# AbnerVictor/OOD-GAN-inversion

Hardware: AMD Instinct MI355X
Metric: 1024² face inversions/sec (100 W+ steps) (higher is better)
Workload: dtype f16-split (hi+lo f16 operands, f32 accumulate): 3 MFMA/product in every forward conv (fp32-equivalent), 2 in the input-gradient convs (back-propagated gradient rounded to f16 before each contraction, weights keep hi+lo); dL/dW+ vs the float64 reference 1.4e-5..3.6e-5 ('f16s': 1.3e-5..2.6e-5, the ref

## Files before the change

include/oodgan.h:

```cpp
#ifndef OODGAN_H
#define OODGAN_H

#ifdef __cplusplus
extern "C" {
#endif

#define OODGAN_OK 0
#define OODGAN_E_ARG (-1)
#define OODGAN_E_LAUNCH (-2)
#define OODGAN_E_STATE (-3)
#define OODGAN_E_NODEV (-4)

int oodgan_version(void);
const char* oodgan_last_error(void);
int oodgan_device_count(void);
int oodgan_set_tunable(const char* name, long value);
long oodgan_get_tunable(const char* name);
long oodgan_dispatch_count(const char* name);
int oodgan_dispatch_reset(void);
int oodgan_zero(void* p, long bytes, void* stream);

void* oodgan_plan_create(void);
int oodgan_plan_destroy(void* plan);
int oodgan_plan_record_begin(void* plan);
// ... 100 lines not shown
    const float* noise_w;
    const float* bias;
    const float* dscale;
    const float* mul2;
    void* ys;
    float* part_r;
    float* part_t;
    float* part_max;
    int s_rgb_stride, noise_batch, dscale_stride;
    float rgb_scale;
    long nmax;
    int ys_hi_only;
} oodgan_actbwd_fuse;

int oodgan_conv3x3(const oodgan_conv_args* args, void* stream);

long oodgan_pack_conv3x3_f16s_bytes(int Co, int Ci, int transpose);
int oodgan_pack_conv3x3_f16s(const float* w, void* wpk16, float* unscale2, int Co, int Ci, float scale, int transpose,
                             int flip, void* stream);
int oodgan_conv3x3_f16s(const oodgan_conv_args* args, const float* unscale2, void* stream);
int oodgan_conv3x3_f16s_nparts(int mode, int Hin, int Win);
int oodgan_conv3x3_f16s_nparts2(int mode, int Hin, int Win, int x_sform);
int oodgan_conv3x3_s2_fuse_supported(int B, int K, int M, int Hin, int Win);
int oodgan_conv3x3_s2_grouped_supported(int B, int K, int M, int groups, int Hin, int Win);
int oodgan_conv3x3_s1_actgrad_supported(int B, int K, int M, int H, int W);
int oodgan_conv3x3_s1_ys_supported(int B, int K, int M, int H, int W);
int oodgan_conv3x3_xf_supported(int B, int K, int M, int H, int W);
int oodgan_conv3x3_xf_nparts(int B, int H, int W);
long oodgan_conv3x3_tiny_workspace(int mode, int B, int K, int M, int Hin, int Win);

#define OODGAN_VMAX_SLOTS 64
long oodgan_sform_bytes(int B, int C, int H, int W);
int oodgan_to_sform(const float* x, const float* scale, int scale_stride, const float* shift, int shift_stride,
                    const float* mul2, void* out, int B, int C, int H, int W, int in_pitch, unsigned* vmax, void* stream);
long oodgan_sform_phases_bytes(int B, int C, int H, int W);
int oodgan_from_sform(const void* xs, const float* scale, int scale_stride, float* y, int B, int C, int H, int W, void* stream);
int oodgan_blurT_to_sform_phases(const float* g, const float* kernel, const float* scale, int scale_stride,
                                 const float* mul2, void* out, int B, int C, int H, int W, void* stream);
int oodgan_to_sform_phases(const float* x, const float* scale, int scale_stride, const float* mul2, void* out, int B,
                           int C, int H, int W, int in_pitch, void* stream);
int oodgan_to_sform_phases_padtl(const float* x, const float* scale, int scale_stride, const float* mul2, void* out, int B,
                                 int C, int H, int W, int in_pitch, void* stream);
int oodgan_conv3x3_nparts(int mode, int Hin, int Win);
int oodgan_absmax_scaled(const float* x, const float* s, int s_stride, unsigned* vmax, int B, int C, long HW, void* stream);
int oodgan_fwd_range_update(unsigned* vmax, float* q, int* flag, int n, void* stream);
int oodgan_fwd_range_plan(const float* s_all, const float* d_all, const int* row_layer, const int* drow_layer, const float* q,
                          float* s_sc, float* d_sc, int B, int R, int DR, int row0, int nrows, int drow0, int ndrows,
                          void* stream);

int oodgan_blur_act_sform(const float* z, const float* kernel, float* y, void* ys, const float* ys_scale, int ys_scale_stride,
                          const float* bias, const float* noise, int noise_batch, const float* noise_w, int act, int B, int C,
                          int H, int W, int in_pitch, unsigned* vmax, void* stream);
int oodgan_blur_act_fform(const float* z, const float* kernel, float* y, const float* ys_scale, int ys_scale_stride,
                          const float* bias, const float* noise, int noise_batch, const float* noise_w, int act,
                          int B, int C, int H, int W, int in_pitch, unsigned* vmax, int kernel_rank_one, void* stream);
int oodgan_upconv_vblur_supported(int B, int K, int M, int H, int W);
int oodgan_upconv_vblur_fform(const void* xs, const void* wpk2, long wset_bytes, const float* unscale4, const float* kh4,
                              const float* out_scale, int out_scale_stride, const float* bias, const float* noise, int noise_batch,
                              const float* noise_w, int act, const float* ys_scale, int ys_scale_stride, unsigned* vmax, float* y,
                              int B, int K, int M, int H, int W, void* stream);
int oodgan_blur_act_sform_sep(const float* z, const float* kernel, float* y, void* ys, const float* ys_scale, int ys_scale_stride,
                              const float* bias, const float* noise, int noise_batch, const float* noise_w, int act, int B, int C,
                              int H, int W, int in_pitch, unsigned* vmax, int kernel_rank_one, void* stream);

int oodgan_act_bwd_sform_nparts(int H, int W);
int oodgan_act_bwd_sform(const float* g_feat, const float* out, const float* noise, int noise_batch, const float* noise_w,
                         const float* bias, const float* g_rgb, const float* w_rgb, const float* s_rgb, int s_rgb_stride,
                         float rgb_scale, const float* dscale, int dscale_stride, const float* mul2, void* ys, float* part_r,
                         float* part_t, float* part_max, int B, int C, int H, int W, void* stream);
int oodgan_act_bwd_sform_f(const float* out_f, const float* noise, int noise_batch, const float* noise_w, const float* bias,
                           const float* g_rgb, const float* w_rgb, const float* s_rgb, int s_rgb_stride, float rgb_scale,
                           const float* dscale, int dscale_stride, const float* mul2, void* ys, float* part_r, float* part_t,
                           float* part_max, int B, int C, int H, int W, void* stream);
int oodgan_from_fform(const float* f, float* y, int B, int C, int H, int W, void* stream);
int oodgan_act_bwd_blurT_nparts(int H, int W);
int oodgan_act_bwd_blurT_pre_supported(int H, int W);
int oodgan_act_bwd_blurT_sform_phases(const float* g_feat, const float* out, const float* noise, int noise_batch,
                                      const float* noise_w, const float* bias, const float* g_rgb, const float* w_rgb,
                                      const float* s_rgb, int s_rgb_stride, float rgb_scale, const float* dscale,
                                      int dscale_stride, const float* mul2, const float* kernel, void* out_phases,
                                      float* part_r, float* part_t, float* part_max, int B, int C, int H, int W, void* stream);
int oodgan_act_bwd_blurT_hi_supported(int H, int W);
int oodgan_conv3x3_s1_xh_supported(int B, int K, int M, int H, int W);
int oodgan_act_bwd_blurT_sform_phases_hi(const float* g_feat, const float* out, const float* noise, int noise_batch, const float* noise_w,
                                         const float* bias, const float* dscale, int dscale_stride, const float* mul2, const float* kernel,
                                         void* out_phases, float* part_r, float* part_max, int B, int C, int H, int W, void* stream);
int oodgan_absmax_scale_check(const float* part, long n, float* state, int* flag, void* stream);

typedef struct oodgan_reduce_job {
    const float* part;
    float* out;
    int B, C, nparts, out_stride, accumulate;
    const float* part2;
    const float* scale2;
    int nparts2, scale2_stride;
} oodgan_reduce_job;
typedef struct oodgan_demod_bwd_job {
    const float* s; const float* wsq; const float* d; const float* r; float* gs;
    int s_stride, d_stride, gs_stride, B, Ci, Co;
    float scale;
} oodgan_demod_bwd_job;
typedef struct oodgan_demod_fwd_job {
    const float* s; const float* wsq; float* d;
    int s_stride, d_stride, B, Ci, Co;
    float scale;
} oodgan_demod_fwd_job;
typedef struct oodgan_scale_check_job {
    const float* part; long n; float* state;
} oodgan_scale_check_job;
int oodgan_reduce_batch(const oodgan_reduce_job* jobs, int njobs, void* stream);
int oodgan_demod_bwd_batch(const oodgan_demod_bwd_job* jobs, int njobs, void* stream);
int oodgan_demod_fwd_batch(const oodgan_demod_fwd_job* jobs, int njobs, void* stream);
int oodgan_absmax_scale_check_batch(const oodgan_scale_check_job* jobs, int njobs, int* flag, void* stream);

long oodgan_hform_bytes(int B, int C, int H, int W);
int oodgan_to_hform(const float* x, void* out, int B, int C, int H, int W, void* stream);
int oodgan_from_hform(const void* in, float* y, int B, int C, int H, int W, void* stream);
long oodgan_modconv_f16_wbytes(int B, int M, int K);
int oodgan_modconv_f16_pack(const float* weight, const float* style, int style_stride, float scale, int demodulate,
                            int act, void* wpk, int B, int M, int K, void* stream);
int oodgan_modconv_f16_pack_affine(const float* weight, const float* latent, int latent_stride, const float* mod_weight,
                                   const float* mod_bias, int S, float scale, int demodulate, int act, void* wpk, int B, int M,
                                   int K, void* stream);
int oodgan_modconv_f16(const void* x, const void* wpk, const float* noise, int noise_batch, const float* noise_w,
                       const float* bias, int act, void* y, int B, int K, int M, int H, int W, void* stream);
int oodgan_reduce_parts(const float* part, float* out, long rows, int nparts, int accumulate, void* stream);
int oodgan_reduce_parts_cols(const float* part, float* out, int B, int C, int nparts, int out_stride, int accumulate,
                             void* stream);


int oodgan_torgb_fwd(const float* x, const float* w, const float* s, int s_stride, const float* bias,
                     const float* skip, const float* kernel, float* y, int B, int Ci, int H, int W,
                     float scale, void* stream);
int oodgan_torgb_fwd_sform(const float* x, const float* w, const float* s, int s_stride, const float* bias,
                           const float* skip, const float* kernel, float* y, void* ys, const float* ys_scale,
                           int ys_scale_stride, int B, int Ci, int H, int W, float scale, unsigned* vmax, void* stream);
int oodgan_rgb_finish(const float* partial, const float* bias, const float* skip, const float* kernel, float* y, int B, int H,
                      int W, void* stream);
int oodgan_rgb_finish_parts(const float* partial, int nparts, const float* bias, const float* skip, const float* kernel, float* y, int B,
                            int H, int W, void* stream);

int oodgan_feature_modulation(const float* x, const float* c0, const float* c1, float* y, long n, int mode, void* stream);

int oodgan_act_bwd_fused(const float* g_feat, const float* out, const float* noise, int noise_batch,
                         const float* noise_w, const float* bias, const float* g_rgb, const float* w_rgb,
                         const float* s_rgb, int s_rgb_stride, float rgb_scale, float* g_pre,
                         float* part_r, float* part_rgb, int B, int C, long HW, void* stream);
int oodgan_act_bwd_nparts(long HW);
int oodgan_act_bwd_fused_max(const float* g_feat, const float* out, const float* noise, int noise_batch,
                             const float* noise_w, const float* bias, const float* g_rgb, const float* w_rgb,
                             const float* s_rgb, int s_rgb_stride, float rgb_scale, float* g_pre,
                             float* part_r, float* part_rgb, float* part_max, const float* dscale, int dscale_stride, int B,
                             int C, long HW, void* stream);
int oodgan_absmax_scale(const float* part, long n, float* out2, void* stream);
int oodgan_absmax_scale_clear(float* part, long n, float* out2, void* stream);


int oodgan_mse_fwd_bwd(const float* img, const float* target, float* gimg, float* part, float* loss,
                       int B, long CHW, float grad_mul, void* stream);
int oodgan_mse_nparts(long CHW);
int oodgan_mse_fwd_bwd_row(const float* img, const float* target, float* gimg, float* part, float* loss_table,
                           const int* row_dev, int nrows, int B, long CHW, float grad_mul, void* stream);
int oodgan_composite_mse_fwd_bwd(const float* img, const float* target, const float* beta, float* gimg, float* comp, float* part,
                                 float* loss, int B, int C, long HW, int wrt_gen, float grad_mul, void* stream);
int oodgan_composite_mse_fwd_bwd_row(const float* img, const float* target, const float* beta, float* gimg, float* comp, float* part,
                                     float* loss_table, const int* row_dev, int nrows, int B, int C, long HW, int wrt_gen,
// ... 83 lines not shown
```

ood-gan-inversion_amd/csrc/common.hpp:

```cpp
#pragma once
#include <hip/hip_runtime.h>
#include <cstdio>
#include <cstdarg>
#include <functional>
#include <utility>
#include "../../include/oodgan.h"

namespace oodgan {
struct PlanRec;
extern thread_local PlanRec* tl_plan_rec;
extern int g_null_launch;
void plan_append(std::function<void()>&& f);
template <class F>
inline void launch_rec(F&& f) {
    f();
    if (__builtin_expect(tl_plan_rec != nullptr, 0)) plan_append(std::function<void()>(std::forward<F>(f)));
}
}
#undef hipLaunchKernelGGL
#define hipLaunchKernelGGL(kernelName, numBlocks, numThreads, memPerBlock, streamId, ...)                                        \
    ::oodgan::launch_rec([=]() {                                                                                                 \
        if (!::oodgan::g_null_launch) (kernelName)<<<(numBlocks), (numThreads), (memPerBlock), (streamId)>>>(__VA_ARGS__);      \
    })

namespace oodgan {

void set_error(const char* fmt, ...);

enum { OODGAN_TUN_S1_BIG_MIN_ITEMS = 0, OODGAN_TUN_S2_BIG_MIN_ITEMS, OODGAN_TUN_T2_BIG_MIN_ITEMS, OODGAN_TUN_BLURT_STRIP, OODGAN_TUN_BLUR_STRIP, OODGAN_TUN_UPVB_WAVES, OODGAN_TUN_FEWOUT_QUAD, OODGAN_TUN_TINY_MID_MAX, OODGAN_TUN_STRIPX_WAVES, OODGAN_TUN_COUNT };
long tunable(int id);

enum { OODGAN_DC_STRIPX = 0, OODGAN_DC_STRIP, OODGAN_DC_S1BIG, OODGAN_DC_S1V2, OODGAN_DC_S1PP, OODGAN_DC_TINY, OODGAN_DC_T2BIG,
       OODGAN_DC_T2V2, OODGAN_DC_T2GEN, OODGAN_DC_S2BIG, OODGAN_DC_S2V2, OODGAN_DC_S2GEN, OODGAN_DC_UPVB,
       OODGAN_DC_S1BIG_YS, OODGAN_DC_S2BIG_FUSE, OODGAN_DC_S2BIG_DOTXS,
       OODGAN_DC_S1BIG_G2, OODGAN_DC_S2BIG_G2, OODGAN_DC_STRIPX_G2, OODGAN_DC_S2BIG_XH, OODGAN_DC_S1BIG_XH,
       OODGAN_DC_COMPOSITE_MSE,
       OODGAN_DC_SSIM,
       OODGAN_DC_ROBUST,
       OODGAN_DC_AREA_POOL, OODGAN_DC_COUNT };
void count_dispatch(int id);

bool bound_device_ok(const char* what);

inline int check_launch(const char* what) {
    hipError_t e = hipGetLastError();
    if (e != hipSuccess) {
        set_error("%s: %s", what, hipGetErrorString(e));
        return OODGAN_E_LAUNCH;
    }
    return OODGAN_OK;
}

#define OODGAN_REQUIRE(cond, ...)          \
    do {                                    \
        if (!(cond)) {                      \
            oodgan::set_error(__VA_ARGS__); \
            return OODGAN_E_ARG;            \
        }                                   \
    } while (0)

constexpr float kSqrt2 = 1.4142135623730951f;
constexpr float kInvPos = 1.f / kSqrt2, kInvNeg = 1.f / (0.2f * kSqrt2);
constexpr int kWave = 64;

inline hipStream_t as_stream(void* s) { return reinterpret_cast<hipStream_t>(s); }

inline int stream_grid(long work_items, int block) {
    long g = (work_items + block - 1) / block;
    if (g > 2048) g = 2048;
    if (g < 1) g = 1;
    return static_cast<int>(g);
}

__device__ __forceinline__ float wave_sum(float v) {
#pragma unroll
    for (int o = 32; o > 0; o >>= 1) v += __shfl_xor(v, o, 64);
    return v;
}

__device__ __forceinline__ float row_sum16(const float* __restrict__ p, int n, int l) {
    float v[4];
#pragma unroll
    for (int u = 0; u < 4; ++u) v[u] = p[min(l + 16 * u, n - 1)];
#pragma unroll
    for (int u = 0; u < 4; ++u) v[u] = l + 16 * u < n ? v[u] : 0.f;
    float r = (v[0] + v[1]) + (v[2] + v[3]);
    r += __shfl_xor(r, 8, 64);
    r += __shfl_xor(r, 4, 64);
    r += __shfl_xor(r, 2, 64);
    r += __shfl_xor(r, 1, 64);
    return r;
}

__device__ __forceinline__ float row_sum_wave(const float* __restrict__ p, int n, int lane) {
    float a0 = 0.f, a1 = 0.f, a2 = 0.f, a3 = 0.f;
    for (int i0 = lane; i0 < n; i0 += 512) {
        float v[8];
#pragma unroll
        for (int u = 0; u < 8; ++u) v[u] = p[min(i0 + 64 * u, n - 1)];
#pragma unroll
        for (int u = 0; u < 8; ++u) v[u] = i0 + 64 * u < n ? v[u] : 0.f;
        a0 += v[0] + v[4]; a1 += v[1] + v[5]; a2 += v[2] + v[6]; a3 += v[3] + v[7];
    }
    return wave_sum((a0 + a1) + (a2 + a3));
}

__device__ __forceinline__ float row_sum(const float* __restrict__ p, int n, int lane) {
    return n <= 64 ? row_sum16(p, n, lane & 15) : row_sum_wave(p, n, lane);
}

__device__ __forceinline__ float demod_dot(const float* __restrict__ sp, const float* __restrict__ wp, int Ci, int lane) {
    float a0 = 0.f, a1 = 0.f, a2 = 0.f, a3 = 0.f;
    for (int c0 = lane; c0 < Ci; c0 += 512) {
        float sv[8], wv[8];
#pragma unroll
        for (int u = 0; u < 8; ++u) {
            const int ci = min(c0 + 64 * u, Ci - 1);
            sv[u] = sp[ci];
            wv[u] = wp[ci];
        }
#pragma unroll
        for (int u = 0; u < 8; ++u) {
// ... 78 lines not shown
```

ood-gan-inversion_amd/csrc/conv_f16s.hip:

```cpp
#include "conv_common.hpp"
#include <cstdlib>
#include <cstdint>

extern "C" int oodgan_conv3x3_f16s_nparts(int mode, int Hin, int Win);

using namespace oodgan;

namespace oodgan {
int launch_s1pp(const oodgan_conv_args& a, const void* wpk16, const float* unscale, hipStream_t st);
int launch_s1v2(const oodgan_conv_args& a, const void* wpk16, const float* unscale, hipStream_t st);
bool s1_strip_eligible(const oodgan_conv_args& a);
bool s1_big_eligible(const oodgan_conv_args& a);
int launch_s1_big(const oodgan_conv_args& a, const void* wpk16, const float* unscale, hipStream_t st);
int launch_s1_strip(const oodgan_conv_args& a, const void* wpk16, const float* unscale, hipStream_t st);
int launch_s1_stripx(const oodgan_conv_args& a, const void* wpk16, const float* unscale, hipStream_t st);
bool tiny_eligible(const oodgan_conv_args& a);
int launch_tiny(const oodgan_conv_args& a, const void* wpk16, const float* unscale, hipStream_t st);
int launch_t2v2(const oodgan_conv_args& a, const void* wpk16, const float* unscale, hipStream_t st);
int launch_s2v2(const oodgan_conv_args& a, const void* wpk16, const float* unscale, hipStream_t st);
bool s2_big_eligible(const oodgan_conv_args& a);
bool t2_big_eligible(const oodgan_conv_args& a);
int launch_t2_big(const oodgan_conv_args& a, const void* wpk16, const float* unscale, hipStream_t st);
int launch_s2_big(const oodgan_conv_args& a, const void* wpk16, const float* unscale, hipStream_t st);
}
// ... 311 lines not shown
}

__global__ __launch_bounds__(256) void pack_f16s_kernel(const float* __restrict__ w, _Float16* __restrict__ out, int Co, int Ci,
                                                        int Mp, float scale, int transpose, int flip,
                                                        const float* __restrict__ sc2) {
    const int K = transpose ? Co : Ci, M = transpose ? Ci : Co;
    const int nchunk = (K + CK - 1) / CK;
    const long total = (long)nchunk * 9 * 2 * Mp * 8;
    const float s2 = sc2[1] * scale;
    for (long e = blockIdx.x * 256L + threadIdx.x; e < total; e += (long)gridDim.x * 256) {
        const int j = (int)(e & 7);
        long r = e >> 3;
        const int m = (int)(r % Mp); r /= Mp;
        const int h = (int)(r & 1); r >>= 1;
        const int tap = (int)(r % 9);
        const int t = (int)(r / 9);
        const int k = t * CK + 8 * h + j;
        float v = 0.f;
        if (m < M && k < K) {
            const int co = transpose ? k : m, ci = transpose ? m : k;
            v = w[((long)co * Ci + ci) * 9 + (flip ? 8 - tap : tap)] * s2;
        }
        const _Float16 hi = (_Float16)v;
        const _Float16 lo = (_Float16)(v - (float)hi);
        const long base = (((long)t * 9 + tap) * 2) * 2;
        out[((base + 0 * 2 + h) * Mp + m) * 8 + j] = hi;
        out[((base + 1 * 2 + h) * Mp + m) * 8 + j] = lo;
    }
}

}

extern "C" int oodgan_conv3x3_f16s_nparts2(int mode, int Hin, int Win, int x_sform) {
    if (mode == OODGAN_CONV_S2 && x_sform) return (((Hin - 1) / 2 + 7) / 8) * (((Win - 1) / 2 + 31) / 32);
    return oodgan_conv3x3_f16s_nparts(mode, Hin, Win);
}

extern "C" int oodgan_conv3x3_f16s_nparts(int mode, int Hin, int Win) {
    if (mode == OODGAN_CONV_S1) return ((Hin + 7) / 8) * ((Win + 31) / 32) ;
    if (mode == OODGAN_CONV_S2) return (((Hin - 1) / 2 + 7) / 8) * (((Win - 1) / 2 + 31) / 32) * 4;
    return 0;
}

extern "C" long oodgan_pack_conv3x3_f16s_bytes(int Co, int Ci, int transpose) {
    const int M = transpose ? Ci : Co, K = transpose ? Co : Ci;
    const long Mp = (M + 63) / 64 * 64;
    return (long)((K + CK - 1) / CK) * 9 * 2 * 2 * Mp * 16;
}

extern "C" int oodgan_pack_conv3x3_f16s(const float* w, void* wpk16, float* unscale2, int Co, int Ci, float scale, int transpose,
                                        int flip, void* stream) {
    OODGAN_REQUIRE(w && wpk16 && unscale2 && Co > 0 && Ci > 0, "pack_conv3x3_f16s: bad args");
    const int M = transpose ? Ci : Co, K = transpose ? Co : Ci;
    const int Mp = (M + 63) / 64 * 64;
    hipStream_t st = as_stream(stream);
    if (hipMemsetAsync(unscale2, 0, 2 * sizeof(float), st) != hipSuccess) {
        set_error("pack_conv3x3_f16s: memset failed");
        return OODGAN_E_LAUNCH;
    }
    hipLaunchKernelGGL(absmax_kernel, dim3(stream_grid((long)Co * Ci * 9, 256 * 16)), dim3(256), 0, st, w, (long)Co * Ci * 9, scale, unscale2);
    hipLaunchKernelGGL(absmax_finish_kernel, dim3(1), dim3(1), 0, st, unscale2);
    const long total = (long)((K + CK - 1) / CK) * 9 * 2 * Mp * 8;
    hipLaunchKernelGGL(pack_f16s_kernel, dim3(stream_grid(total, 256)), dim3(256), 0, st, w, reinterpret_cast<_Float16*>(wpk16),
                       Co, Ci, Mp, scale, transpose, flip, unscale2);
    return check_launch("pack_conv3x3_f16s");
}

extern "C" int oodgan_conv3x3_s1_actgrad_supported(int B, int K, int M, int H, int W) {
    oodgan_conv_args a = {};
    a.mode = OODGAN_CONV_S1; a.x_sform = 1; a.B = B; a.K = K; a.M = M; a.Hin = H; a.Win = W;
    a.y = reinterpret_cast<float*>(1);
    a.dotx = reinterpret_cast<const float*>(1);
    return (s1_strip_eligible(a) || s1_big_eligible(a)) && oodgan_act_bwd_blurT_pre_supported(H / 2, W / 2) && !(H & 1) && !(W & 1) ? 1 : 0;
}

extern "C" int oodgan_conv3x3_s1_xh_supported(int B, int K, int M, int H, int W) {
    oodgan_conv_args a = {};
    a.mode = OODGAN_CONV_S1; a.x_sform = 1; a.B = B; a.K = K; a.M = M; a.Hin = H; a.Win = W;
    a.y = reinterpret_cast<float*>(1);
    a.dotx = reinterpret_cast<const float*>(1);
    return (H > 8 && W > 8 && !s1_strip_eligible(a) && s1_big_eligible(a)) ? 1 : 0;
}

extern "C" int oodgan_conv3x3_s1_ys_supported(int B, int K, int M, int H, int W) {
    oodgan_conv_args a = {};
    a.mode = OODGAN_CONV_S1; a.x_sform = 1; a.B = B; a.K = K; a.M = M; a.Hin = H; a.Win = W;
    a.ys = reinterpret_cast<void*>(1);
    return s1_big_eligible(a) ? 1 : 0;
}

extern "C" int oodgan_conv3x3_f16s(const oodgan_conv_args* args, const float* unscale2, void* stream) {
    OODGAN_REQUIRE(args != nullptr, "conv3x3_f16s: null args");
    const oodgan_conv_args& a = *args;
    OODGAN_REQUIRE(a.x && a.wpk && unscale2 && (a.y || a.x_sform), "conv3x3_f16s: null tensor");
    OODGAN_REQUIRE(a.B > 0 && a.K > 0 && a.M > 0 && a.Hin > 0 && a.Win > 0, "conv3x3_f16s: bad shape");
    OODGAN_REQUIRE(a.act != OODGAN_ACT_PRELU || a.slope, "conv3x3_f16s: PReLU without slopes");
    OODGAN_REQUIRE(a.noise == nullptr || a.noise_batch == 1 || a.noise_batch == a.B, "conv3x3_f16s: noise_batch");
    if (!bound_device_ok("conv3x3_f16s")) return OODGAN_E_ARG;
    if (a.x_fform) {
        OODGAN_REQUIRE(a.x_fform == 1 || a.x_fform == 2, "conv3x3_f16s: x_fform must be 0, 1 or 2");
        count_dispatch(OODGAN_DC_STRIPX);
        return launch_s1_stripx(a, a.wpk, unscale2, as_stream(stream));
    }
    OODGAN_REQUIRE(!a.dotx_fform, "conv3x3_f16s: an F-form dotx exists only with x_fform == 2");
    OODGAN_REQUIRE(a.rgb_y == nullptr || (a.mode == OODGAN_CONV_S1 && a.x_sform), "conv3x3_f16s: fused ToRGB output only for mode S1 with S-form input");
    OODGAN_REQUIRE(a.fuse == nullptr || (a.mode == OODGAN_CONV_S2 && a.x_sform && a.M >= 64),
                   "conv3x3_f16s: the fused activation backward exists only for mode S2 with S-form input and M >= 64");
    OODGAN_REQUIRE(a.groups <= 1 || (a.mode == OODGAN_CONV_S2 && (!a.x_sform || tiny_eligible(a) || s2_big_eligible(a))),
                   "conv3x3_f16s: groups > 1 only for mode S2 with fp32 NCHW input, or a phase-split S-form input of a shape the 8-wave or the skinny-GEMM kernel "
                   "takes (oodgan_conv3x3_s2_grouped_supported; oodgan_conv3x3_tiny_workspace > 0 with a workspace)");
    OODGAN_REQUIRE(!a.y_fform || (a.mode == OODGAN_CONV_S1 && a.x_sform && s1_strip_eligible(a)),
                   "conv3x3_f16s: the F-form output exists only in the strip kernel (mode S1, S-form input, 16 < K,M <= 32)");
    OODGAN_REQUIRE(!a.dot_actgrad || (a.mode == OODGAN_CONV_S1 && a.x_sform && a.dotx && (s1_strip_eligible(a) || s1_big_eligible(a))),
                   "conv3x3_f16s: dot_actgrad exists only in the strip / 8-wave kernels of mode S1 (oodgan_conv3x3_s1_actgrad_supported)");
    OODGAN_REQUIRE(!a.dotx_sform || (a.mode == OODGAN_CONV_S2 && a.x_sform && a.fuse && a.dotx && a.dotx_scale && a.dotx_scale_stride >= a.M &&
                                     !tiny_eligible(a) && s2_big_eligible(a)),
                   "conv3x3_f16s: dotx_sform needs mode S2, a phase-split S-form input, `fuse`, dotx, dotx_scale and a shape of the 8-wave kernel "
                   "(oodgan_conv3x3_s2_fuse_supported)");
    OODGAN_REQUIRE(a.ys_vmax == nullptr || (a.ys != nullptr && a.mode == OODGAN_CONV_S1 && a.x_sform && !tiny_eligible(a) && !s1_strip_eligible(a) && s1_big_eligible(a)),
                   "conv3x3_f16s: ys_vmax only with ys from the 8-wave stride-1 kernel (oodgan_conv3x3_s1_ys_supported)");
    OODGAN_REQUIRE(a.x_hi_only != 2 || (a.x_sform && a.dotx && !tiny_eligible(a) &&
                                        ((a.mode == OODGAN_CONV_S2 && s2_big_eligible(a)) || (a.mode == OODGAN_CONV_S1 && !s1_strip_eligible(a) && s1_big_eligible(a)))),
                   "conv3x3_f16s: x_hi_only = 2 (32-byte hi-only input records) exists only in the two-instruction 8-wave kernels (S-form input, dotx; mode S2 on a "
                   "shape oodgan_conv3x3_s2_fuse_supported accepts, mode S1 on a shape of the 8-wave stride-1 kernel)");
    hipStream_t st = as_stream(stream);
    switch (a.mode) {
        case OODGAN_CONV_S1:
            if (tiny_eligible(a)) { count_dispatch(OODGAN_DC_TINY); return launch_tiny(a, a.wpk, unscale2, st); }
            if (a.x_sform && s1_strip_eligible(a)) { count_dispatch(OODGAN_DC_STRIP); return launch_s1_strip(a, a.wpk, unscale2, st); }
            if (a.x_sform && s1_big_eligible(a)) { count_dispatch(OODGAN_DC_S1BIG); if (a.ys) count_dispatch(OODGAN_DC_S1BIG_YS); return launch_s1_big(a, a.wpk, unscale2, st); }
            OODGAN_REQUIRE(a.rgb_y == nullptr, "conv3x3_f16s: the fused ToRGB output exists only in the strip kernel (16 < K,M <= 32) and, as partial "
                                               "sums together with ys, in the 8-wave kernel (oodgan_conv3x3_s1_ys_supported)");
            if (a.x_sform) { count_dispatch(OODGAN_DC_S1V2); return launch_s1v2(a, a.wpk, unscale2, st); }
            OODGAN_REQUIRE(a.ys == nullptr, "conv3x3_f16s: S-form output needs the S-form input kernel");
            count_dispatch(OODGAN_DC_S1PP);
            return launch_s1pp(a, a.wpk, unscale2, st);
        case OODGAN_CONV_T2:
            if (a.x_sform && t2_big_eligible(a)) { count_dispatch(OODGAN_DC_T2BIG); return launch_t2_big(a, a.wpk, unscale2, st); }
            if (a.x_sform) { count_dispatch(OODGAN_DC_T2V2); return launch_t2v2(a, a.wpk, unscale2, st); }
            count_dispatch(OODGAN_DC_T2GEN);
            return launch_mode<OODGAN_CONV_T2>(a, a.wpk, unscale2, st);
        case OODGAN_CONV_S2:
            OODGAN_REQUIRE((a.Hin & 1) && (a.Win & 1) && a.Hin >= 3 && a.Win >= 3, "conv3x3_f16s S2: input must be odd-sized");
            if (tiny_eligible(a)) { count_dispatch(OODGAN_DC_TINY); return launch_tiny(a, a.wpk, unscale2, st); }
            if (a.x_sform && s2_big_eligible(a)) { count_dispatch(OODGAN_DC_S2BIG); if (a.fuse) count_dispatch(OODGAN_DC_S2BIG_FUSE); if (a.dotx_sform) count_dispatch(OODGAN_DC_S2BIG_DOTXS); return launch_s2_big(a, a.wpk, unscale2, st); }
            if (a.x_sform) { count_dispatch(OODGAN_DC_S2V2); return launch_s2v2(a, a.wpk, unscale2, st); }
            count_dispatch(OODGAN_DC_S2GEN);
            return launch_mode<OODGAN_CONV_S2>(a, a.wpk, unscale2, st);
        default: break;
    }
    set_error("conv3x3_f16s: unknown mode %d", a.mode);
    return OODGAN_E_ARG;
}
```

ood-gan-inversion_amd/csrc/conv_f16s_big.hip:

```cpp
#include "conv_common.hpp"
#include "sform.hpp"
#include <cstdint>
#include <cstdlib>
#include <type_traits>

using namespace oodgan;

typedef _Float16 half8 __attribute__((ext_vector_type(8)));
typedef __attribute__((address_space(3))) void lds_void;

namespace {

constexpr int BG_R = 18, BG_C = 34;
constexpr int BG_XSLOTS = BG_R * BG_C * 4;
constexpr int BG_XPIECES = (BG_XSLOTS + 63) / 64;
constexpr int BG_XBYTES = BG_XPIECES * 1024;
constexpr int BG_WPIECES = 36;
constexpr int BG_STAGE = BG_XBYTES + BG_WPIECES * 1024;
constexpr int BG_PIECES = BG_XPIECES + BG_WPIECES;
constexpr int BG_RED = 2 * BG_STAGE;
constexpr int BG_SMEM = BG_RED + 8 * 64 * 4;

struct BigConv {
    oodgan_conv_args a;
    const uint4* xs;
    SDims xd;
    const float* w_unscale;
    int tiles_x, tiles_y, mblocks, Mp;
    long out_plane;
    SDims yd;
};

constexpr int BG_ZERO = BG_SMEM;
constexpr int BG_ZBYTES = 3584;
constexpr int BG_CST = BG_SMEM + BG_ZBYTES;
constexpr int BG_NZ = BG_CST + 3 * 64 * 4;
constexpr int BG_RGBW = BG_NZ + 2048;
constexpr int BG_SMEM16 = BG_RGBW + 3 * 64 * 4;
typedef float f32x4v __attribute__((ext_vector_type(4)));

#ifdef OODGAN_CLOCK_STAMP
__device__ unsigned long long* g_s1big_stamp = nullptr;
__device__ long g_s1big_stamp_n = 0;
#endif

template <bool DOT, bool PRE, bool YS = false, bool G2 = false>
__global__ __launch_bounds__(512) void conv_f16s_s1big_kernel(const BigConv p, const uint4* __restrict__ wpk16) {
    constexpr int NW = 8, NT = 2;
    extern __shared__ __attribute__((aligned(16))) unsigned char smem[];
    const oodgan_conv_args& a = p.a;
    const int tid = threadIdx.x, lane = tid & 63;
    const int wave = __builtin_amdgcn_readfirstlane(tid >> 6);
    const int n16 = lane & 15, g = lane >> 4;

    int w = xcd_remap(blockIdx.x, gridDim.x);
    const int mblk = w % p.mblocks;
    w /= p.mblocks;
    const int ntile = p.tiles_x * p.tiles_y;
    const int tile = w % ntile, b = w / ntile;
    const int ty = tile / p.tiles_x, tx = tile % p.tiles_x;
    const int r0 = ty * 16, c0 = tx * 32, m0 = mblk * 64;
    const int H = a.Hin, W = a.Win, M = a.M;

    constexpr int NPW = (BG_PIECES + NW - 1) / NW;
    unsigned off[NPW];
    const bool xh = G2 && a.x_hi_only == 2;
    unsigned xmask = 0;
    const int KC = p.xd.KC;
#pragma unroll
    for (int i = 0; i < NPW; ++i) {
        const int pc = wave + NW * i;
        if (pc < BG_XPIECES) {
            int P = pc * 64 + lane;
            if (P >= BG_XSLOTS) P = BG_XSLOTS - 1;
            const int row = P / (BG_C * 4), q = P % (BG_C * 4);
            const int c = q >> 2, sl = ((q & 3) - 2 * ((c >> 2) & 1)) & 3;
            const int rr = min(r0 + row, p.xd.Hp - 1);
            if (xh) {
                off[i] = (unsigned)((((long)rr * p.xd.Wp + (c0 + c)) * 2 + (sl & 1)) * 16);
                if (sl < 2) xmask |= 1u << i;
            } else {
                off[i] = (unsigned)((((long)rr * p.xd.Wp + (c0 + c)) * 4 + sl) * 16);
                xmask |= 1u << i;
            }
        } else {
            xmask |= 1u << i;
            const int u = (pc - BG_XPIECES) * 64 + lane;
            const int row = u >> 6, j = u & 63;
            off[i] = (unsigned)((((long)row * p.Mp) + m0 + j) * 16);
        }
    }
    const unsigned char* xb = reinterpret_cast<const unsigned char*>(p.xs) + (long)b * KC * p.xd.plane * 16;
    const long xplane_bytes = p.xd.plane * 16;
    const unsigned char* wb = reinterpret_cast<const unsigned char*>(wpk16);
    const long wchunk_bytes = (long)36 * p.Mp * 16;
    const int nchunk = (a.K + 15) / 16;
    auto dma_piece = [&](int t, int buf, int i) {
        const int pc = wave + NW * i;
        if (pc >= BG_PIECES) return;
        unsigned char* dst = smem + buf * BG_STAGE;
        const unsigned char* src = (pc < BG_XPIECES ? xb + (long)t * xplane_bytes : wb + (long)t * wchunk_bytes) + off[i];
        if (!G2 || ((xmask >> i) & 1u))
            __builtin_amdgcn_global_load_lds((const __attribute__((address_space(1))) void*)src, (lds_void*)(dst + pc * 1024), 16, 0, 0);
    };
    for (int i = tid; i < BG_ZBYTES / 16; i += 512) reinterpret_cast<uint4*>(smem + BG_ZERO)[i] = make_uint4(0, 0, 0, 0);
    __syncthreads();

    f32x4v acc[4][4];
#pragma unroll
    for (int mt = 0; mt < 4; ++mt)
#pragma unroll
        for (int n = 0; n < 4; ++n) acc[mt][n] = f32x4v{0.f, 0.f, 0.f, 0.f};

    const unsigned laneA = (unsigned)((((g & 1) * 64 + n16) * 16) + (g >> 1) * 4096);
    const unsigned laneA1 = (unsigned)(((g & 1) * 64 + n16) * 16);
    unsigned offBh[4], offBl[4];
#pragma unroll
    for (int pp = 0; pp < 4; ++pp) {
        const int tp = 2 * pp + (g >> 1), ky = tp / 3, kx = tp % 3, col = n16 + kx;
        offBh[pp] = (unsigned)(ky * (BG_C * 64) + col * 64 + ((((g & 1) + 2 * ((col >> 2) & 1)) & 3) << 4));
        offBl[pp] = (unsigned)(ky * (BG_C * 64) + col * 64 + ((((g & 1) + 2 + 2 * ((col >> 2) & 1)) & 3) << 4));
    }
    const int col8 = n16 + 2;
    const unsigned offB1 = (unsigned)(2 * (BG_C * 64) + col8 * 64 + ((((G2 ? (g & 1) : g) + 2 * ((col8 >> 2) & 1)) & 3) << 4));

    struct AF { half8 x[2], y[2]; };
    struct BF { half8 u[4], v[4]; };
    auto load_a = [&](AF& f, const unsigned char* lw, auto pp_c, auto mh_c) {
        constexpr int pp = decltype(pp_c)::value, mh = decltype(mh_c)::value;
        const unsigned char* q = lw + (pp < 4 ? laneA + 2 * pp * 4096 : laneA1 + 8 * 4096 + (G2 ? (g >> 1) * 2048 : 0));
#pragma unroll
        for (int i = 0; i < 2; ++i) {
            f.x[i] = *reinterpret_cast<const half8*>(q + (2 * mh + i) * 256);
            if (!(G2 && pp == 4)) f.y[i] = *reinterpret_cast<const half8*>(q + 2048 + (2 * mh + i) * 256);
        }
    };
    auto load_b = [&](BF& f, const unsigned char* lx, const unsigned char* lz, auto pp_c, auto part_c) {
        constexpr int pp = decltype(pp_c)::value, part = decltype(part_c)::value;
#pragma unroll
        for (int n = 0; n < 4; ++n) {
            const int o = (n >> 1) * (BG_C * 64) + (n & 1) * 1024;
            if (G2) {
                if (part == 0) f.u[n] = *reinterpret_cast<const half8*>(lx + (pp < 4 ? offBh[pp < 4 ? pp : 0] : offB1) + o);
            } else if (pp < 4) {
                if (part == 0) f.u[n] = *reinterpret_cast<const half8*>(lx + offBh[pp < 4 ? pp : 0] + o);
                else f.v[n] = *reinterpret_cast<const half8*>(lx + offBl[pp < 4 ? pp : 0] + o);
            } else {
                if (part == 0) f.u[n] = *reinterpret_cast<const half8*>(lx + offB1 + o);
                else f.v[n] = *reinterpret_cast<const half8*>(lz + o);
            }
        }
    };
    auto mfma_half = [&](const AF& fa, const BF& fb, auto pp_c, auto mh_c) {
        constexpr int pp = decltype(pp_c)::value, mh = decltype(mh_c)::value;
        if (G2) {
#pragma unroll
            for (int i = 0; i < 2; ++i)
#pragma unroll
                for (int n = 0; n < 4; ++n) acc[2 * mh + i][n] = __builtin_amdgcn_mfma_f32_16x16x32_f16(fa.x[i], fb.u[n], acc[2 * mh + i][n], 0, 0, 0);
            if (pp < 4) {
#pragma unroll
                for (int i = 0; i < 2; ++i)
#pragma unroll
                    for (int n = 0; n < 4; ++n) acc[2 * mh + i][n] = __builtin_amdgcn_mfma_f32_16x16x32_f16(fa.y[i], fb.u[n], acc[2 * mh + i][n], 0, 0, 0);
            }
        } else if (pp < 4) {
#pragma unroll
            for (int i = 0; i < 2; ++i)
#pragma unroll
                for (int n = 0; n < 4; ++n) acc[2 * mh + i][n] = __builtin_amdgcn_mfma_f32_16x16x32_f16(fa.x[i], fb.u[n], acc[2 * mh + i][n], 0, 0, 0);
#pragma unroll
            for (int i = 0; i < 2; ++i)
#pragma unroll
                for (int n = 0; n < 4; ++n) acc[2 * mh + i][n] = __builtin_amdgcn_mfma_f32_16x16x32_f16(fa.x[i], fb.v[n], acc[2 * mh + i][n], 0, 0, 0);
#pragma unroll
            for (int i = 0; i < 2; ++i)
#pragma unroll
                for (int n = 0; n < 4; ++n) acc[2 * mh + i][n] = __builtin_amdgcn_mfma_f32_16x16x32_f16(fa.y[i], fb.u[n], acc[2 * mh + i][n], 0, 0, 0);
        } else {
#pragma unroll
            for (int i = 0; i < 2; ++i)
#pragma unroll
                for (int n = 0; n < 4; ++n) acc[2 * mh + i][n] = __builtin_amdgcn_mfma_f32_16x16x32_f16(fa.x[i], fb.u[n], acc[2 * mh + i][n], 0, 0, 0);
#pragma unroll
            for (int i = 0; i < 2; ++i)
#pragma unroll
                for (int n = 0; n < 4; ++n) acc[2 * mh + i][n] = __builtin_amdgcn_mfma_f32_16x16x32_f16(fa.y[i], fb.v[n], acc[2 * mh + i][n], 0, 0, 0);
        }
    };
#define BH_IC(n) std::integral_constant<int, n>{}
#define BH_SB() __builtin_amdgcn_sched_barrier(0)
#ifdef OODGAN_CLOCK_STAMP
    const unsigned long long st_t0 = __builtin_amdgcn_s_memtime(), st_r0 = __builtin_amdgcn_s_memrealtime();
#endif
    float cst_o = 0.f, cst_b = 0.f, cst_s = 1.f, rgb_c0 = 0.f, rgb_c1 = 0.f, rgb_c2 = 0.f;
    if (tid < 64 && m0 + tid < M) {
        const int m = m0 + tid;
        cst_o = a.out_scale ? a.out_scale[(long)b * a.out_scale_stride + m] : 1.f;
        if (!DOT && a.bias) cst_b = a.bias[m];
        if (!DOT && a.act == OODGAN_ACT_PRELU) cst_s = a.slope[m];
        if (YS && a.rgb_y) {
            const float sv = a.rgb_scale * a.rgb_s[(long)b * a.rgb_s_stride + m];
            rgb_c0 = sv * a.rgb_w[m]; rgb_c1 = sv * a.rgb_w[M + m]; rgb_c2 = sv * a.rgb_w[2 * M + m];
        }
    }
    const bool has_nz = !DOT && a.noise != nullptr;
    if (has_nz) {
        const int ry = min(r0 + wave * NT + (lane >> 5), H - 1), rx = min(c0 + (lane & 31), W - 1);
        const float* src = a.noise + (long)(a.noise_batch > 1 ? b : 0) * H * W + (long)ry * W + rx;
        __builtin_amdgcn_global_load_lds((const __attribute__((address_space(1))) void*)src, (lds_void*)(smem + BG_NZ + wave * 256), 4, 0, 0);
    }
#pragma unroll
    for (int i = 0; i < NPW; ++i) dma_piece(0, 0, i);
    if (tid < 64) {
        float* cst = reinterpret_cast<float*>(smem + BG_CST);
        cst[tid] = cst_o;
        if (!DOT) { cst[64 + tid] = cst_b; cst[128 + tid] = cst_s; }
        if (YS) {
            float* rw = reinterpret_cast<float*>(smem + BG_RGBW);
            rw[tid] = rgb_c0; rw[64 + tid] = rgb_c1; rw[128 + tid] = rgb_c2;
        }
        __builtin_amdgcn_s_waitcnt(0xC07F);
    }
    for (int t = 0; t < nchunk; ++t) {
        __builtin_amdgcn_s_waitcnt(0x0F70);
        __builtin_amdgcn_s_barrier();
        const bool pf = t + 1 < nchunk;
        const int nb = (t + 1) & 1;
        const unsigned char* lx = smem + (t & 1) * BG_STAGE + (wave * NT) * (BG_C * 64);
        const unsigned char* lw = smem + (t & 1) * BG_STAGE + BG_XBYTES;
        const unsigned col8r = (unsigned)(2 * (BG_C * 64) + col8 * 64 + ((((g & 1) + 2 * ((col8 >> 2) & 1)) & 3) << 4));
        const unsigned char* lz = g < 2 ? lx + col8r : smem + BG_ZERO;
        AF a0, a1;
        BF b0, b1;
#define BH_DMA(i) if (pf && (i) < NPW) dma_piece(t + 1, nb, (i));
        load_b(b0, lx, lz, BH_IC(0), BH_IC(0)); load_b(b0, lx, lz, BH_IC(0), BH_IC(1));
        load_a(a0, lw, BH_IC(0), BH_IC(0));
        BH_SB();
        load_a(a1, lw, BH_IC(0), BH_IC(1)); load_b(b1, lx, lz, BH_IC(1), BH_IC(0)); BH_DMA(0) BH_SB(); mfma_half(a0, b0, BH_IC(0), BH_IC(0)); BH_SB();
        load_a(a0, lw, BH_IC(1), BH_IC(0)); load_b(b1, lx, lz, BH_IC(1), BH_IC(1)); BH_DMA(1) BH_SB(); mfma_half(a1, b0, BH_IC(0), BH_IC(1)); BH_SB();
        load_a(a1, lw, BH_IC(1), BH_IC(1)); load_b(b0, lx, lz, BH_IC(2), BH_IC(0)); BH_DMA(2) BH_SB(); mfma_half(a0, b1, BH_IC(1), BH_IC(0)); BH_SB();
        load_a(a0, lw, BH_IC(2), BH_IC(0)); load_b(b0, lx, lz, BH_IC(2), BH_IC(1)); BH_DMA(3) BH_SB(); mfma_half(a1, b1, BH_IC(1), BH_IC(1)); BH_SB();
        load_a(a1, lw, BH_IC(2), BH_IC(1)); load_b(b1, lx, lz, BH_IC(3), BH_IC(0)); BH_DMA(4) BH_SB(); mfma_half(a0, b0, BH_IC(2), BH_IC(0)); BH_SB();
        load_a(a0, lw, BH_IC(3), BH_IC(0)); load_b(b1, lx, lz, BH_IC(3), BH_IC(1)); BH_DMA(5) BH_SB(); mfma_half(a1, b0, BH_IC(2), BH_IC(1)); BH_SB();
        load_a(a1, lw, BH_IC(3), BH_IC(1)); load_b(b0, lx, lz, BH_IC(4), BH_IC(0)); BH_DMA(6) BH_SB(); mfma_half(a0, b1, BH_IC(3), BH_IC(0)); BH_SB();
        load_a(a0, lw, BH_IC(4), BH_IC(0)); load_b(b0, lx, lz, BH_IC(4), BH_IC(1)); BH_DMA(7) BH_SB(); mfma_half(a1, b1, BH_IC(3), BH_IC(1)); BH_SB();
        load_a(a1, lw, BH_IC(4), BH_IC(1)); BH_DMA(8) BH_SB(); mfma_half(a0, b0, BH_IC(4), BH_IC(0)); BH_SB();
        BH_DMA(9) BH_SB();
        mfma_half(a1, b0, BH_IC(4), BH_IC(1));
#undef BH_DMA
    }
#undef BH_IC
#undef BH_SB
#ifdef OODGAN_CLOCK_STAMP
    if (tid == 0 && g_s1big_stamp && (long)blockIdx.x < g_s1big_stamp_n) {
        g_s1big_stamp[2 * blockIdx.x] = __builtin_amdgcn_s_memtime() - st_t0;
        g_s1big_stamp[2 * blockIdx.x + 1] = __builtin_amdgcn_s_memrealtime() - st_r0;
    }
#endif

    const float us = (p.w_unscale ? p.w_unscale[0] : 1.f) * (a.in_mul2 ? a.in_mul2[0] : 1.f);
    const float nw = (!DOT && a.noise) ? (a.noise_w ? a.noise_w[0] : 1.f) : 0.f;
    float* red = reinterpret_cast<float*>(smem + BG_RED);
    float osc[16], bia[16], slp[16];
    unsigned moff[16], doff[16];
    float dsum[16];
    const bool prelu = !DOT && a.act == OODGAN_ACT_PRELU;
    const float* cst = reinterpret_cast<const float*>(smem + BG_CST);
#pragma unroll
    for (int q = 0; q < 16; ++q) {
        const int j = 16 * (q >> 2) + 4 * g + (q & 3), m = m0 + j;
        const bool mok = m < M;
        osc[q] = cst[j] * us;
        bia[q] = DOT ? 0.f : cst[64 + j];
        slp[q] = DOT ? 1.f : cst[128 + j];
        moff[q] = mok ? (unsigned)((long)m * p.out_plane * 4) : 0xFFFFFFFFu;
        doff[q] = mok ? (unsigned)((long)m * H * W * 4) : 0u;
        dsum[q] = 0.f;
    }
    const bool mfull = m0 + 64 <= M;
    float ysc[16], ysmax = 0.f;
    if (YS) {
#pragma unroll
        for (int q = 0; q < 16; ++q) {
            const int m = m0 + 16 * (q >> 2) + 4 * g + (q & 3);
            ysc[q] = a.ys_scale ? a.ys_scale[(long)b * a.ys_scale_stride + min(m, M - 1)] : 1.f;
        }
    }
#pragma unroll
    for (int n = 0; n < 4; ++n) {
        const int py = r0 + wave * NT + (n >> 1), px = c0 + 16 * (n & 1) + n16;
        const bool ok = py < H && px < W;
        float nz = 0.f;
        if (has_nz) nz = nw * reinterpret_cast<const float*>(smem + BG_NZ)[wave * 64 + (n >> 1) * 32 + 16 * (n & 1) + n16];
        unsigned char* yr = reinterpret_cast<unsigned char*>(a.y) + ((long)b * M * p.out_plane + (long)py * a.out_pitch + px) * 4;
        const unsigned char* dr = DOT ? reinterpret_cast<const unsigned char*>(a.dotx) + ((long)b * M * H * W + (long)py * W + px) * 4 : nullptr;
        float o[16], dv[16];
        if (DOT) {
#pragma unroll
            for (int q = 0; q < 16; ++q) dv[q] = 0.f;
            if (ok) {
                if (mfull) {
#pragma unroll
                    for (int q = 0; q < 16; ++q) dv[q] = *reinterpret_cast<const float*>(dr + doff[q]);
                } else {
#pragma unroll
                    for (int q = 0; q < 16; ++q)
                        if (moff[q] != 0xFFFFFFFFu) dv[q] = *reinterpret_cast<const float*>(dr + doff[q]);
                }
            }
        }
#pragma unroll
        for (int q = 0; q < 16; ++q) {
            const float v = acc[q >> 2][n][q & 3];
            o[q] = v * osc[q];
            if (DOT) {
                dsum[q] += (v * us) * dv[q];
                if (PRE) o[q] *= dv[q] > 0.f ? kSqrt2 : 0.2f * kSqrt2;
            } else {
                o[q] += nz + bia[q];
                if (a.act == OODGAN_ACT_LRELU) o[q] = (o[q] > 0.f ? o[q] : 0.2f * o[q]) * kSqrt2;
                else if (prelu) o[q] = o[q] > 0.f ? o[q] : slp[q] * o[q];
            }
        }
        if (ok && (!YS || a.y != nullptr)) {
            if (mfull) {
#pragma unroll
                for (int q = 0; q < 16; ++q) *reinterpret_cast<float*>(yr + moff[q]) = o[q];
            } else {
#pragma unroll
                for (int q = 0; q < 16; ++q)
                    if (moff[q] != 0xFFFFFFFFu) *reinterpret_cast<float*>(yr + moff[q]) = o[q];
            }
        }
        if (YS && !DOT && ok) {
#pragma unroll
            for (int mt = 0; mt < 4; ++mt) {
                if (m0 + 16 * mt < M) {
                    const float v0 = o[4 * mt] * ysc[4 * mt], v1 = o[4 * mt + 1] * ysc[4 * mt + 1], v2 = o[4 * mt + 2] * ysc[4 * mt + 2],
                                v3 = o[4 * mt + 3] * ysc[4 * mt + 3];
                    ysmax = fmaxf(fmaxf(ysmax, fmaxf(fabsf(v0), fabsf(v1))), fmaxf(fabsf(v2), fabsf(v3)));
                    uint2 hi, lo;
                    split_pair(v0, v1, hi.x, lo.x);
                    split_pair(v2, v3, hi.y, lo.y);
                    unsigned char* rec = reinterpret_cast<unsigned char*>(a.ys) + sform_unit(p.yd, b, (m0 >> 4) + mt, py, px, g >> 1) * 16 + (g & 1) * 8;
                    *reinterpret_cast<uint2*>(rec) = hi;
                    *reinterpret_cast<uint2*>(rec + 32) = lo;
                }
            }
        }
        if (YS && !DOT && a.rgb_y) {
            const float* rw = reinterpret_cast<const float*>(smem + BG_RGBW);
            float c0 = 0.f, c1 = 0.f, c2 = 0.f;
#pragma unroll
            for (int q = 0; q < 16; ++q) {
                const int j = 16 * (q >> 2) + 4 * g + (q & 3);
                c0 += rw[j] * o[q]; c1 += rw[64 + j] * o[q]; c2 += rw[128 + j] * o[q];
            }
            c0 += __shfl_xor(c0, 16, 64); c1 += __shfl_xor(c1, 16, 64); c2 += __shfl_xor(c2, 16, 64);
            c0 += __shfl_xor(c0, 32, 64); c1 += __shfl_xor(c1, 32, 64); c2 += __shfl_xor(c2, 32, 64);
            if (ok && g == 0) {
                float* rp = a.rgb_y + (((long)mblk * a.B + b) * 3) * ((long)H * W) + (long)py * W + px;
                rp[0] = c0; rp[(long)H * W] = c1; rp[2 * (long)H * W] = c2;
            }
        }
    }
    if (YS && a.ys_vmax) record_vmax(a.ys_vmax, b, ysmax);
    if (DOT) {
#pragma unroll
        for (int q = 0; q < 16; ++q) {
            float v = dsum[q];
            v += dpp_take<0xB1, 0xF>(v);
            v += dpp_take<0x4E, 0xF>(v);
            v += dpp_take<0x141, 0xF>(v);
            v += dpp_take<0x140, 0xF>(v);
            if (n16 == 0) red[wave * 64 + 16 * (q >> 2) + 4 * g + (q & 3)] = v;
        }
        __syncthreads();
        if (tid < 64 && m0 + tid < M) {
            float v = 0.f;
#pragma unroll
            for (int wv = 0; wv < NW; ++wv) v += red[wv * 64 + tid];
            float* dp = a.dot_part + ((long)b * M + m0 + tid) * a.dot_nparts;
            const int tx8 = (W + 31) / 32;
            dp[(long)(2 * ty) * tx8 + tx] = v;
            if (2 * ty + 1 < (H + 7) / 8) dp[(long)(2 * ty + 1) * tx8 + tx] = 0.f;
        }
    }
}

}

namespace oodgan {

bool s1_big_eligible(const oodgan_conv_args& a) {
    const int min_k = 64;
    if (!(a.mode == OODGAN_CONV_S1 && a.x_sform && a.K >= min_k && a.M >= 64 && (a.ys == nullptr ? (a.y != nullptr && a.rgb_y == nullptr) : (a.dotx == nullptr && a.M % 16 == 0)) &&
          (a.act == OODGAN_ACT_NONE || a.act == OODGAN_ACT_LRELU || (a.act == OODGAN_ACT_PRELU && a.slope)) && a.in_scale == nullptr &&
          a.in_shift == nullptr &&
          !(a.dotx && (a.noise || a.bias || a.act != OODGAN_ACT_NONE))))
        return false;
    const long items = (long)((a.Hin + 15) / 16) * ((a.Win + 31) / 32) * a.B * ((a.M + 63) / 64);
    return items >= tunable(OODGAN_TUN_S1_BIG_MIN_ITEMS);
}

int launch_s1_big(const oodgan_conv_args& a_in, const void* wpk16, const float* unscale, hipStream_t st) {
    BigConv p;
    p.a = a_in;
    oodgan_conv_args& a = p.a;
    if (a.out_pitch == 0) a.out_pitch = a.Win;
    p.out_plane = (long)a.Hin * a.out_pitch;
    p.xs = reinterpret_cast<const uint4*>(a.x);
    p.xd = sform_dims(a.K, a.Hin, a.Win);
    p.w_unscale = unscale;
    p.tiles_y = (a.Hin + 15) / 16;
    p.tiles_x = (a.Win + 31) / 32;
    p.Mp = (a.M + 63) / 64 * 64;
    p.mblocks = (a.M + 63) / 64;
    p.yd = sform_dims(a.M, a.Hin, a.Win);
    if (a.dotx) {
        OODGAN_REQUIRE(a.dot_part != nullptr, "conv3x3: dotx without dot_part");
        OODGAN_REQUIRE(a.dot_nparts == ((a.Hin + 7) / 8) * p.tiles_x, "conv3x3 f16s S1: dot_nparts %d != %d", a.dot_nparts,
                       ((a.Hin + 7) / 8) * p.tiles_x);
    }
    OODGAN_REQUIRE((long)a.M * p.out_plane * 4 < (1L << 32) && (long)a.M * a.Hin * a.Win * 4 < (1L << 32), "conv3x3 big: plane too large");
    const long total = (long)p.tiles_x * p.tiles_y * a.B * p.mblocks;
    OODGAN_REQUIRE(total > 0 && total < (1L << 31), "conv3x3: grid too large");
    static bool once = ((void)hipFuncSetAttribute(reinterpret_cast<const void*>(&conv_f16s_s1big_kernel<true, false>), hipFuncAttributeMaxDynamicSharedMemorySize, BG_SMEM16),
                        (void)hipFuncSetAttribute(reinterpret_cast<const void*>(&conv_f16s_s1big_kernel<true, true>), hipFuncAttributeMaxDynamicSharedMemorySize, BG_SMEM16),
                        (void)hipFuncSetAttribute(reinterpret_cast<const void*>(&conv_f16s_s1big_kernel<false, false>), hipFuncAttributeMaxDynamicSharedMemorySize, BG_SMEM16),
                        (void)hipFuncSetAttribute(reinterpret_cast<const void*>(&conv_f16s_s1big_kernel<false, false, true>), hipFuncAttributeMaxDynamicSharedMemorySize, BG_SMEM16),
                        (void)hipFuncSetAttribute(reinterpret_cast<const void*>(&conv_f16s_s1big_kernel<true, false, false, true>), hipFuncAttributeMaxDynamicSharedMemorySize, BG_SMEM16),
                        (void)hipFuncSetAttribute(reinterpret_cast<const void*>(&conv_f16s_s1big_kernel<true, true, false, true>), hipFuncAttributeMaxDynamicSharedMemorySize, BG_SMEM16), true);
    (void)once;
    const uint4* w16 = reinterpret_cast<const uint4*>(wpk16);
    OODGAN_REQUIRE(!a.dot_actgrad || a.dotx, "conv3x3 big: dot_actgrad without dotx");
    const bool g2 = a.x_hi_only != 0 && a.dotx != nullptr;
    OODGAN_REQUIRE(a.x_hi_only != 2 || g2, "conv3x3 big: hi-only input records (x_hi_only = 2) need dotx (the two-instruction instances)");
    if (g2) count_dispatch(OODGAN_DC_S1BIG_G2);
    if (g2 && a.x_hi_only == 2) count_dispatch(OODGAN_DC_S1BIG_XH);
    if (a.dot_actgrad && g2) hipLaunchKernelGGL((conv_f16s_s1big_kernel<true, true, false, true>), dim3((unsigned)total), dim3(512), BG_SMEM16, st, p, w16);
    else if (g2) hipLaunchKernelGGL((conv_f16s_s1big_kernel<true, false, false, true>), dim3((unsigned)total), dim3(512), BG_SMEM16, st, p, w16);
    else if (a.dot_actgrad) hipLaunchKernelGGL((conv_f16s_s1big_kernel<true, true>), dim3((unsigned)total), dim3(512), BG_SMEM16, st, p, w16);
    else if (a.dotx) hipLaunchKernelGGL((conv_f16s_s1big_kernel<true, false>), dim3((unsigned)total), dim3(512), BG_SMEM16, st, p, w16);
    else if (a.ys) hipLaunchKernelGGL((conv_f16s_s1big_kernel<false, false, true>), dim3((unsigned)total), dim3(512), BG_SMEM16, st, p, w16);
    else hipLaunchKernelGGL((conv_f16s_s1big_kernel<false, false>), dim3((unsigned)total), dim3(512), BG_SMEM16, st, p, w16);
    return check_launch("conv3x3_f16s_s1big");
}

}

#ifdef OODGAN_CLOCK_STAMP
extern "C" int oodgan_debug_set_stamp_buffer(void* buf, long n) {
    unsigned long long* p = reinterpret_cast<unsigned long long*>(buf);
    if (hipMemcpyToSymbol(HIP_SYMBOL(g_s1big_stamp), &p, sizeof(p)) != hipSuccess ||
        hipMemcpyToSymbol(HIP_SYMBOL(g_s1big_stamp_n), &n, sizeof(n)) != hipSuccess) {
        oodgan::set_error("debug_set_stamp_buffer: hipMemcpyToSymbol failed");
        return OODGAN_E_LAUNCH;
    }
    return 0;
}
#endif
```

ood-gan-inversion_amd/csrc/fwd_producers.hip:

```cpp
#include "common.hpp"
#include "sform.hpp"
#include <cstdint>

using namespace oodgan;

typedef _Float16 half2v __attribute__((ext_vector_type(2)));
typedef _Float16 half8 __attribute__((ext_vector_type(8)));

namespace {

constexpr int FT_R = 11, FT_C = 72;
constexpr int FT_P = 74, FT_Q = 816;
constexpr int LS_ROW = 65, LS_CH = 520;

__device__ __forceinline__ bool tile_elem(int k, int i, int& r, int& c4) {
    if (k < FT_R) { r = k; c4 = i; return true; }
    r = i; c4 = 16 + (k - FT_R);
    return i < FT_R;
}

struct BlurArgs {
    const float* z;
    const float* kern;
    float* y;
// ... 52 lines not shown
            const int gy = Y0 - 1 + r, gx = X0 - 4 + 4 * c4;
            v[k] = make_float4(0.f, 0.f, 0.f, 0.f);
            if (act && c < a.C && gy >= 0 && gy < Hz && gx >= 0 && gx + 3 < a.pitch)
                v[k] = *reinterpret_cast<const float4*>(zp + (long)gy * a.pitch + gx);
        }
#pragma unroll
        for (int k = 0; k < NE; ++k) {
            int r, c4;
            if (!tile_elem(k, tid & 15, r, c4)) continue;
            const int gx = X0 - 4 + 4 * c4;
            if (gx + 3 >= Wz) {
                if (gx + 0 >= Wz) v[k].x = 0.f;
                if (gx + 1 >= Wz) v[k].y = 0.f;
                if (gx + 2 >= Wz) v[k].z = 0.f;
                v[k].w = 0.f;
            }
            float2* dst = reinterpret_cast<float2*>(lin + ch * FT_Q + r * FT_P + 4 * c4);
            dst[0] = make_float2(v[k].x, v[k].y);
            dst[1] = make_float2(v[k].z, v[k].w);
        }
    }
    __syncthreads();
    const int ch = tid >> 4, tq = tid & 15;
    const int yrow = tq >> 1, xh = tq & 1;
    float o[32];
    if (ksep[8] != 0.f) {
#pragma unroll
        for (int hf = 0; hf < 2; ++hf) {
            float tmp[20];
#pragma unroll
            for (int j = 0; j < 20; ++j) tmp[j] = 0.f;
#pragma unroll
            for (int aa = 0; aa < 4; ++aa) {
                const float2* row = reinterpret_cast<const float2*>(lin + ch * FT_Q + (yrow + aa) * FT_P + 32 * xh + 16 * hf + 2);
                const float kv = ksep[aa];
#pragma unroll
                for (int j = 0; j < 10; ++j) {
                    const float2 v = row[j];
                    tmp[2 * j] += kv * v.x;
                    tmp[2 * j + 1] += kv * v.y;
                }
            }
#pragma unroll
            for (int j = 0; j < 16; ++j)
                o[16 * hf + j] = ksep[4] * tmp[j + 1] + ksep[5] * tmp[j + 2] + ksep[6] * tmp[j + 3] + ksep[7] * tmp[j + 4];
        }
    } else {
#pragma unroll
        for (int j = 0; j < 32; ++j) o[j] = 0.f;
#pragma unroll
        for (int aa = 0; aa < 4; ++aa) {
            const float* row = lin + ch * FT_Q + (yrow + aa) * FT_P + 32 * xh + 3;
            float win[35];
#pragma unroll
            for (int j = 0; j < 35; ++j) win[j] = row[j];
#pragma unroll
            for (int bb = 0; bb < 4; ++bb) {
                const float kv = kf[aa * 4 + bb];
#pragma unroll
                for (int j = 0; j < 32; ++j) o[j] += kv * win[j + bb];
            }
        }
    }
    __syncthreads();
    float* lst = lin;
#pragma unroll
    for (int j = 0; j < 32; ++j) lst[ch * LS_CH + yrow * LS_ROW + 32 * xh + j] = o[j];
    __syncthreads();
    const float nw = a.noise ? (a.noise_w ? a.noise_w[0] : 1.f) : 0.f;
    const long HWo = (long)Ho * Wo;
    float vm = 0.f;
#pragma unroll
    for (int rep = 0; rep < 2; ++rep) {
        const int pos = tid + rep * 256;
        const int Y = Y0 + (pos >> 6), X = X0 + (pos & 63);
        if (Y >= Ho || X >= Wo) continue;
        const float nz = a.noise ? nw * a.noise[(long)(a.noise_batch > 1 ? b : 0) * HWo + (long)Y * Wo + X] : 0.f;
        float* yp = a.y + ((long)b * a.C + kc * 16) * HWo + (long)Y * Wo + X;
#pragma unroll
        for (int cc = 0; cc < 16; ++cc) {
            float* cell = &lst[cc * LS_CH + (pos >> 6) * LS_ROW + (pos & 63)];
            float t = *cell + nz + cb[0][cc];
            if (a.act == OODGAN_ACT_LRELU) t = (t > 0.f ? t : 0.2f * t) * kSqrt2;
            if (!a.y_fform && kc * 16 + cc < a.C) yp[(long)cc * HWo] = t;
            const float v = t * cb[1][cc];
            vm = fmaxf(vm, fabsf(v));
            *cell = a.y_fform ? t : v;
        }
    }
    if (a.y_fform) {
        __syncthreads();
        float* yf = a.y + ((long)b * KC + kc) * HWo * 16;
#pragma unroll
        for (int rep = 0; rep < 8; ++rep) {
            const int u = tid + rep * 256;
            const int pos = u >> 2, q = u & 3;
            const int Y = Y0 + (pos >> 6), X = X0 + (pos & 63);
            if (Y >= Ho || X >= Wo) continue;
            const float* cell = &lst[(4 * q) * LS_CH + (pos >> 6) * LS_ROW + (pos & 63)];
            *reinterpret_cast<float4*>(yf + ((long)Y * Wo + X) * 16 + 4 * q) = make_float4(cell[0], cell[LS_CH], cell[2 * LS_CH], cell[3 * LS_CH]);
        }
    }
    if (a.ys && !a.y_fform) {
        __syncthreads();
#pragma unroll
        for (int rep = 0; rep < 8; ++rep) {
            const int u = tid + rep * 256;
            const int pos = u >> 2, sl = u & 3;
            const int Y = Y0 + (pos >> 6), X = X0 + (pos & 63);
            if (Y >= Ho || X >= Wo) continue;
            half8 o8;
#pragma unroll
            for (int cc = 0; cc < 8; ++cc) {
                const float val = lst[(8 * (sl & 1) + cc) * LS_CH + (pos >> 6) * LS_ROW + (pos & 63)];
                const _Float16 hh = (_Float16)val;
                o8[cc] = (sl & 2) ? (_Float16)(val - (float)hh) : hh;
            }
            reinterpret_cast<half8*>(a.ys + sform_unit(a.yd, b, kc, Y, X, 0))[sl] = o8;
        }
    }
    if (a.vmax) record_vmax(a.vmax, b, vm);
}


struct BlurStripGeo { int nstrips, nseg, seg_rows; };

template <bool SF, bool FULL>
__global__ __launch_bounds__(256) __attribute__((amdgpu_waves_per_eu(4, 8))) void blur_act_fform_strip_kernel(const BlurArgs a, const BlurStripGeo geo) {
    constexpr int GP = 68;
    __shared__ __attribute__((aligned(16))) float gat[2][16][GP];
    const int tid = threadIdx.x;
    int w;
    {
        const int total = gridDim.x, bid = blockIdx.x, xcd = bid & 7, idx = bid >> 3, q = total >> 3, r = total & 7;
        w = (xcd < r ? xcd * (q + 1) : r * (q + 1) + (xcd - r) * q) + idx;
    }
    const int strip = w % geo.nstrips; w /= geo.nstrips;
    const int seg = w % geo.nseg; w /= geo.nseg;
    const int KC = a.yd.KC, kc = w % KC, b = w / KC;
    const int Ho = 2 * a.H, Wo = 2 * a.W, Hz = Ho + 1, Wz = Wo + 1;
    const int Y0 = seg * geo.seg_rows, Y1 = min(Y0 + geo.seg_rows, Ho);
    const int X0 = 64 * strip;
    int pr = 3, pc = 3;
    float k00 = a.kern[15];
    if (!(fabsf(k00) > 0.f)) {
        float best = 0.f;
        for (int i = 0; i < 16; ++i) {
            const float v = fabsf(a.kern[i]);
            if (v > best) { best = v; pr = i >> 2; pc = i & 3; }
        }
        k00 = a.kern[pr * 4 + pc];
    }
    const bool piv = fabsf(k00) > 0.f;
    const float kv0 = piv ? a.kern[12 + pc] / k00 : 0.f, kv1 = piv ? a.kern[8 + pc] / k00 : 0.f, kv2 = piv ? a.kern[4 + pc] / k00 : 0.f,
                kv3 = piv ? a.kern[pc] / k00 : 0.f;
    const float kh0 = a.kern[pr * 4 + 3], kh1 = a.kern[pr * 4 + 2], kh2 = a.kern[pr * 4 + 1], kh3 = a.kern[pr * 4];
    const int ch = tid >> 4, q = tid & 15, c = kc * 16 + ch;
    const float* zp = a.z + ((long)b * a.C + c) * Hz * a.pitch;
    const float bv = a.bias ? a.bias[c] : 0.f;
    const float ysc = a.ys_scale ? a.ys_scale[(long)b * a.ys_scale_stride + c] : 1.f;
    const float nw = a.noise ? (a.noise_w ? a.noise_w[0] : 1.f) : 0.f;
    const long HWo = (long)Ho * Wo;
    const float* np = a.noise ? a.noise + (long)(a.noise_batch > 1 ? b : 0) * HWo : nullptr;
    const int gx = X0 + 4 * q;
    struct Row { float4 m; float e0, e1; float4 n; float rv; };
    const int gxc = min(gx, a.pitch - 4);
    const bool mk0 = gx + 0 < Wz, mk1 = gx + 1 < Wz, mk2 = gx + 2 < Wz, mk3 = gx + 3 < Wz;
    const bool q0 = q == 0, q15 = q == 15;
    const int ec0 = q0 ? max(X0 - 1, 0) : min(X0 + 64, a.pitch - 1), ec1 = min(X0 + 65, a.pitch - 1);
    const bool me0 = q0 ? X0 >= 1 : X0 + 64 < Wz, me1 = X0 + 65 < Wz;
    const bool mkn = np != nullptr && gx + 3 < Wo;
    const int gxn = min(gx, Wo - 4);
    const float* nsrc = np ? np : zp;
    auto load_row = [&](int r, int Y, Row& R) {
        const float* rp = zp + (long)min(max(r, 0), Hz - 1) * a.pitch;
        R.rv = (r >= 0 && r < Hz) ? 1.f : 0.f;
        R.m = *reinterpret_cast<const float4*>(rp + gxc);
        R.e0 = rp[ec0];
        R.e1 = rp[ec1];
        R.n = *reinterpret_cast<const float4*>(nsrc + (long)min(max(Y, 0), Ho - 1) * Wo + gxn);
    };
    auto hpass = [&](const Row& R, float (&h)[4]) {
        const float mx = mk0 ? R.m.x : 0.f, my = mk1 ? R.m.y : 0.f, mz = mk2 ? R.m.z : 0.f, mw = mk3 ? R.m.w : 0.f;
        const float e0 = me0 ? R.e0 : 0.f, e1 = me1 ? R.e1 : 0.f;
        float lw = __builtin_bit_cast(float, __builtin_amdgcn_update_dpp(0, __builtin_bit_cast(int, mw), 0x111, 0xF, 0xF, false));
        float rx = __builtin_bit_cast(float, __builtin_amdgcn_update_dpp(0, __builtin_bit_cast(int, mx), 0x101, 0xF, 0xF, false));
        float ry = __builtin_bit_cast(float, __builtin_amdgcn_update_dpp(0, __builtin_bit_cast(int, my), 0x101, 0xF, 0xF, false));
        if (q0) lw = e0;
        if (q15) { rx = e0; ry = e1; }
        const float x[7] = {lw, mx, my, mz, mw, rx, ry};
#pragma unroll
        for (int e = 0; e < 4; ++e) h[e] = (kh0 * x[e] + kh1 * x[e + 1] + kh2 * x[e + 2] + kh3 * x[e + 3]) * R.rv;
    };

    float h0[4], h1[4], h2[4];
    Row R0, R1, R2;
    R0.n = R1.n = R2.n = make_float4(0.f, 0.f, 0.f, 0.f);
    {
        Row T0, T1, T2;
        T0.n = T1.n = T2.n = make_float4(0.f, 0.f, 0.f, 0.f);
        load_row(Y0 - 1, -1, T0);
        load_row(Y0, -1, T1);
        load_row(Y0 + 1, -1, T2);
        load_row(Y0 + 2, Y0, R0);
        load_row(Y0 + 3, Y0 + 1, R1);
        load_row(Y0 + 4, Y0 + 2, R2);
        hpass(T0, h0);
        hpass(T1, h1);
        hpass(T2, h2);
    }
    float vm = 0.f;
    float* yf = a.y + ((long)b * KC + kc) * HWo * 16;
    float* yplane = a.y + ((long)b * a.C + min(c, a.C - 1)) * HWo;
    const bool yok = c < a.C && gx + 3 < Wo;
    const int pcol = tid >> 2, pq = tid & 3;
    const int sw = ch & 8;
    const bool pok = X0 + pcol < Wo;
    auto step = [&](int Y, Row& R) __attribute__((always_inline)) {
        __builtin_amdgcn_sched_barrier(0);
        float h3[4];
        hpass(R, h3);
        const float nn[4] = {mkn ? R.n.x : 0.f, mkn ? R.n.y : 0.f, mkn ? R.n.z : 0.f, mkn ? R.n.w : 0.f};
        load_row(Y + 5, Y + 3, R);
        float t[4];
#pragma unroll
        for (int e = 0; e < 4; ++e) {
            float v = kv0 * h0[e] + kv1 * h1[e] + kv2 * h2[e] + kv3 * h3[e] + nw * nn[e] + bv;
            if (a.act == OODGAN_ACT_LRELU) v = (v > 0.f ? v : 0.2f * v) * kSqrt2;
            t[e] = v;
            if (gx + e < Wo) vm = fmaxf(vm, fabsf(v * ysc));
            h0[e] = h1[e]; h1[e] = h2[e]; h2[e] = h3[e];
        }
        float (*gb)[GP] = gat[Y & 1];
        if constexpr (SF) {
            if (FULL || yok) *reinterpret_cast<float4*>(yplane + (long)Y * Wo + gx) = make_float4(t[0], t[1], t[2], t[3]);
            *reinterpret_cast<float4*>(&gb[ch][(4 * q) ^ sw]) = make_float4(t[0] * ysc, t[1] * ysc, t[2] * ysc, t[3] * ysc);
            __syncthreads();
            if (FULL || pok) {
                half8 o8;
#pragma unroll
                for (int cc = 0; cc < 8; ++cc) {
                    const float val = gb[8 * (pq & 1) + cc][pcol ^ (8 * (pq & 1))];
                    const _Float16 hh = (_Float16)val;
                    o8[cc] = (pq & 2) ? (_Float16)(val - (float)hh) : hh;
                }
                reinterpret_cast<half8*>(a.ys + sform_unit(a.yd, b, kc, Y, X0 + pcol, 0))[pq] = o8;
            }
        } else {
            *reinterpret_cast<float4*>(&gb[ch][(4 * q) ^ sw]) = make_float4(t[0], t[1], t[2], t[3]);
            __syncthreads();
            if (FULL || pok) {
                const int pc_ = pcol ^ ((pq & 2) << 2);
                *reinterpret_cast<float4*>(yf + ((long)Y * Wo + X0 + pcol) * 16 + 4 * pq) =
                    make_float4(gb[4 * pq][pc_], gb[4 * pq + 1][pc_], gb[4 * pq + 2][pc_], gb[4 * pq + 3][pc_]);
            }
        }
    };
    int Y = Y0;
    for (; Y + 2 < Y1; Y += 3) {
        step(Y, R0);
        step(Y + 1, R1);
        step(Y + 2, R2);
    }
    if (Y < Y1) step(Y, R0);
    if (Y + 1 < Y1) step(Y + 1, R1);
    if (a.vmax && c < a.C) record_vmax(a.vmax, b, vm);
}

}

static int blur_act_launch(const float* z, const float* kernel, float* y, void* ys, const float* ys_scale,
                           int ys_scale_stride, const float* bias, const float* noise, int noise_batch,
                           const float* noise_w, int act, int B, int C, int H, int W, int in_pitch, unsigned* vmax,
                           int y_fform, int rank_one, void* stream) {
    OODGAN_REQUIRE(z && kernel && y && B > 0 && C > 0 && H > 0 && W > 0, "blur_act_sform: bad args");
    OODGAN_REQUIRE(noise == nullptr || noise_batch == 1 || noise_batch == B, "blur_act_sform: noise_batch");
    OODGAN_REQUIRE(act == OODGAN_ACT_NONE || act == OODGAN_ACT_LRELU, "blur_act_sform: act must be none or lrelu");
    if (in_pitch == 0) in_pitch = 2 * W + 1;
    OODGAN_REQUIRE(in_pitch >= 2 * W + 1 && (in_pitch % 4) == 0 && (reinterpret_cast<uintptr_t>(z) & 15) == 0,
                   "blur_act_sform: the input needs 16-byte aligned rows (pitch %% 4 == 0)");
    BlurArgs a;
    a.z = z; a.kern = kernel; a.y = y; a.ys = reinterpret_cast<uint4*>(ys); a.ys_scale = ys_scale;
    a.ys_scale_stride = ys_scale_stride; a.bias = bias; a.noise = noise; a.noise_w = noise_w; a.noise_batch = noise_batch;
    a.act = act; a.B = B; a.C = C; a.H = H; a.W = W; a.pitch = in_pitch;
    a.tiles_x = (2 * W + 63) / 64;
    a.tiles_y = (2 * H + 7) / 8;
    a.yd = sform_dims(C, 2 * H, 2 * W);
    a.vmax = (ys || y_fform) ? vmax : nullptr;
    a.y_fform = y_fform;
    OODGAN_REQUIRE(!y_fform || (C % 16 == 0 && (reinterpret_cast<uintptr_t>(y) & 15) == 0), "blur_act_fform: C %% 16 == 0 and a 16-byte aligned y");
    if ((y_fform || ys) && rank_one == 1 && 2 * W >= 64 && (W % 2) == 0 && (C % 16) == 0 && oodgan::tunable(oodgan::OODGAN_TUN_BLUR_STRIP)) {
        BlurStripGeo geo;
        geo.nstrips = (2 * W + 63) / 64;
        const long base = (long)B * a.yd.KC * geo.nstrips;
        long nseg = (8L * 1024) / base;
        if (nseg < 1) nseg = 1;
        int seg_rows = (int)((2 * H + nseg - 1) / nseg);
        if (seg_rows < 32) seg_rows = 32;
        geo.seg_rows = seg_rows;
        geo.nseg = (2 * H + seg_rows - 1) / seg_rows;
        const long nbs = base * geo.nseg;
        OODGAN_REQUIRE(nbs < (1L << 31), "blur_act_fform: grid too large");
        const bool full = ((2 * W) % 64) == 0;
#define OODGAN_BLUR_STRIP_LAUNCH(SF, FULL) \
    hipLaunchKernelGGL((blur_act_fform_strip_kernel<SF, FULL>), dim3((unsigned)nbs), dim3(256), 0, as_stream(stream), a, geo)
        if (y_fform) { if (full) OODGAN_BLUR_STRIP_LAUNCH(false, true); else OODGAN_BLUR_STRIP_LAUNCH(false, false); }
        else { if (full) OODGAN_BLUR_STRIP_LAUNCH(true, true); else OODGAN_BLUR_STRIP_LAUNCH(true, false); }
#undef OODGAN_BLUR_STRIP_LAUNCH
        return check_launch("blur_act_strip");
    }
    const long nb = (long)a.tiles_x * a.tiles_y * a.yd.KC * B;
    OODGAN_REQUIRE(nb < (1L << 31), "blur_act_sform: grid too large");
    hipLaunchKernelGGL(blur_act_sform_kernel, dim3((unsigned)nb), dim3(256), 0, as_stream(stream), a);
    return check_launch("blur_act_sform");
}

extern "C" int oodgan_blur_act_sform(const float* z, const float* kernel, float* y, void* ys, const float* ys_scale,
                                     int ys_scale_stride, const float* bias, const float* noise, int noise_batch,
                                     const float* noise_w, int act, int B, int C, int H, int W, int in_pitch, unsigned* vmax,
                                     void* stream) {
    return blur_act_launch(z, kernel, y, ys, ys_scale, ys_scale_stride, bias, noise, noise_batch, noise_w, act, B, C, H, W, in_pitch, vmax, 0, 0, stream);
}

extern "C" int oodgan_blur_act_sform_sep(const float* z, const float* kernel, float* y, void* ys, const float* ys_scale,
                                         int ys_scale_stride, const float* bias, const float* noise, int noise_batch,
                                         const float* noise_w, int act, int B, int C, int H, int W, int in_pitch, unsigned* vmax,
                                         int kernel_rank_one, void* stream) {
    return blur_act_launch(z, kernel, y, ys, ys_scale, ys_scale_stride, bias, noise, noise_batch, noise_w, act, B, C, H, W, in_pitch, vmax, 0,
                           kernel_rank_one, stream);
}

extern "C" int oodgan_blur_act_fform(const float* z, const float* kernel, float* y, const float* ys_scale, int ys_scale_stride,
                                     const float* bias, const float* noise, int noise_batch, const float* noise_w, int act,
                                     int B, int C, int H, int W, int in_pitch, unsigned* vmax, int kernel_rank_one, void* stream) {
    return blur_act_launch(z, kernel, y, nullptr, ys_scale, ys_scale_stride, bias, noise, noise_batch, noise_w, act, B, C, H, W, in_pitch, vmax, 1, kernel_rank_one, stream);
}
```

ood-gan-inversion_amd/csrc/runtime.hip:

```cpp
#include "common.hpp"
#include <atomic>
#include <cstdlib>
#include <cstring>
#include <new>

namespace oodgan {
static thread_local char g_err[512] = "";
void set_error(const char* fmt, ...) {
    va_list ap;
    va_start(ap, fmt);
    vsnprintf(g_err, sizeof(g_err), fmt, ap);
    va_end(ap);
}
}

namespace oodgan {
namespace {
struct Tunable { const char* name; const char* env; long def; std::atomic<long> val; std::atomic<int> init; };
Tunable g_tun[OODGAN_TUN_COUNT] = {
    {"s1_big_min_items", "OODGAN_S1_BIG_MIN_ITEMS", 128, {0}, {0}},
    {"s2_big_min_items", "OODGAN_S2_BIG_MIN_ITEMS", 128, {0}, {0}},
    {"t2_big_min_items", "OODGAN_T2_BIG_MIN_ITEMS", 128, {0}, {0}},
    {"blurt_strip", "OODGAN_BLURT_STRIP", 1, {0}, {0}},
    {"blur_strip", "OODGAN_BLUR_STRIP", 1, {0}, {0}},
    {"upvb_waves", "OODGAN_UPVB_WAVES", 12, {0}, {0}},
    {"fewout_quad", "OODGAN_FEWOUT_QUAD", 1, {0}, {0}},
    {"tiny_mid_max", "OODGAN_TINY_MID_MAX", 1024, {0}, {0}},
    {"stripx_waves", "OODGAN_STRIPX_WAVES", 4, {0}, {0}},
};
}
long tunable(int id) {
    Tunable& t = g_tun[id];
    if (!t.init.load(std::memory_order_acquire)) {
        const char* e = getenv(t.env);
        t.val.store(e ? atol(e) : t.def, std::memory_order_relaxed);
        t.init.store(1, std::memory_order_release);
    }
    return t.val.load(std::memory_order_relaxed);
}
}

extern "C" int oodgan_set_tunable(const char* name, long value) {
    OODGAN_REQUIRE(name != nullptr, "set_tunable: null name");
    for (int i = 0; i < oodgan::OODGAN_TUN_COUNT; ++i)
        if (strcmp(name, oodgan::g_tun[i].name) == 0) {
            oodgan::g_tun[i].val.store(value, std::memory_order_relaxed);
            oodgan::g_tun[i].init.store(1, std::memory_order_release);
            return OODGAN_OK;
        }
    oodgan::set_error("set_tunable: unknown tunable '%s'", name);
    return OODGAN_E_ARG;
}
extern "C" long oodgan_get_tunable(const char* name) {
    if (name)
        for (int i = 0; i < oodgan::OODGAN_TUN_COUNT; ++i)
            if (strcmp(name, oodgan::g_tun[i].name) == 0) return oodgan::tunable(i);
    return -1;
}

namespace oodgan {
bool bound_device_ok(const char* what) {
    static std::atomic<int> bound{-1};
    int dev = 0;
    if (hipGetDevice(&dev) != hipSuccess) {
        (void)hipGetLastError();
        set_error("%s: no current HIP device", what);
        return false;
    }
    int expected = -1;
    if (bound.compare_exchange_strong(expected, dev, std::memory_order_acq_rel) || expected == dev) return true;
    set_error("%s: liboodgan_hip.so is bound to HIP device %d (its first use in this process) but device %d is current — one process per GPU "
              "(select the device with HIP_VISIBLE_DEVICES or torch.cuda.set_device before the first call)", what, expected, dev);
    return false;
}
}

namespace oodgan {
namespace {
const char* const g_dc_name[OODGAN_DC_COUNT] = {"stripx", "strip", "s1big", "s1v2", "s1pp", "tiny", "t2big", "t2v2", "t2gen", "s2big", "s2v2", "s2gen", "upvb", "s1big_ys", "s2big_fuse", "s2big_dotx_sform", "s1big_g2", "s2big_g2", "stripx_g2", "s2big_xh", "s1big_xh", "composite_mse", "ssim", "robust", "area_pool"};
std::atomic<long> g_dc[OODGAN_DC_COUNT];
}
void count_dispatch(int id) { g_dc[id].fetch_add(1, std::memory_order_relaxed); }
}
extern "C" long oodgan_dispatch_count(const char* name) {
    if (name)
        for (int i = 0; i < oodgan::OODGAN_DC_COUNT; ++i)
            if (strcmp(name, oodgan::g_dc_name[i]) == 0) return oodgan::g_dc[i].load(std::memory_order_relaxed);
    return -1;
}
extern "C" int oodgan_dispatch_reset(void) {
    for (int i = 0; i < oodgan::OODGAN_DC_COUNT; ++i) oodgan::g_dc[i].store(0, std::memory_order_relaxed);
    return OODGAN_OK;
}

namespace {
__global__ __launch_bounds__(256) void zero_kernel(unsigned char* __restrict__ p, long bytes) {
    const long i = (long)blockIdx.x * 256 + threadIdx.x;
    const long head = (16 - (reinterpret_cast<uintptr_t>(p) & 15)) & 15;
    const long h = head < bytes ? head : bytes;
    const long n16 = (bytes - h) >> 4;
    if (i < n16) reinterpret_cast<uint4*>(p + h)[i] = make_uint4(0u, 0u, 0u, 0u);
    if (i < h) p[i] = 0;
    const long tail = h + (n16 << 4);
    if (i < bytes - tail) p[tail + i] = 0;
}
}

extern "C" int oodgan_zero(void* p, long bytes, void* stream) {
    OODGAN_REQUIRE(p != nullptr && bytes >= 0, "zero: bad args");
    if (bytes == 0) return OODGAN_OK;
    const long items = (bytes >> 4) + 16;
    OODGAN_REQUIRE((items + 255) / 256 < (1L << 31), "zero: too large");
    hipLaunchKernelGGL(zero_kernel, dim3((unsigned)((items + 255) / 256)), dim3(256), 0, oodgan::as_stream(stream),
                       reinterpret_cast<unsigned char*>(p), bytes);
    return oodgan::check_launch("zero");
}

#include <vector>
namespace oodgan {
struct PlanRec {
    std::vector<std::function<void()>> ops;
    bool recording = false;
};
thread_local PlanRec* tl_plan_rec = nullptr;
int g_null_launch = 0;
void plan_append(std::function<void()>&& f) { tl_plan_rec->ops.emplace_back(std::move(f)); }
}

extern "C" void* oodgan_plan_create(void) { return new (std::nothrow) oodgan::PlanRec(); }
extern "C" int oodgan_plan_destroy(void* plan) {
    oodgan::PlanRec* p = static_cast<oodgan::PlanRec*>(plan);
    if (p && oodgan::tl_plan_rec == p) oodgan::tl_plan_rec = nullptr;
    delete p;
    return OODGAN_OK;
}
extern "C" int oodgan_plan_record_begin(void* plan) {
    oodgan::PlanRec* p = static_cast<oodgan::PlanRec*>(plan);
    OODGAN_REQUIRE(p != nullptr, "plan_record_begin: null plan");
    OODGAN_REQUIRE(oodgan::tl_plan_rec == nullptr, "plan_record_begin: this thread is already recording a plan");
    p->ops.clear();
    p->recording = true;
    oodgan::tl_plan_rec = p;
    return OODGAN_OK;
}
extern "C" long oodgan_plan_record_end(void* plan) {
    oodgan::PlanRec* p = static_cast<oodgan::PlanRec*>(plan);
    if (p == nullptr || oodgan::tl_plan_rec != p) {
        oodgan::set_error("plan_record_end: this thread is not recording that plan");
        return -1;
    }
    oodgan::tl_plan_rec = nullptr;
    p->recording = false;
    return (long)p->ops.size();
}
extern "C" long oodgan_plan_size(const void* plan) { return plan ? (long)static_cast<const oodgan::PlanRec*>(plan)->ops.size() : -1; }
extern "C" int oodgan_plan_run(void* plan, int times) {
    oodgan::PlanRec* p = static_cast<oodgan::PlanRec*>(plan);
    OODGAN_REQUIRE(p != nullptr && !p->recording && times >= 0, "plan_run: null plan, a plan still recording, or times < 0");
    OODGAN_REQUIRE(oodgan::tl_plan_rec == nullptr, "plan_run: this thread is recording a plan");
    for (int t = 0; t < times; ++t)
        for (const std::function<void()>& f : p->ops) f();
    return oodgan::check_launch("plan_run");
// ... 17 lines not shown
```

ood-gan-inversion_amd/oodgan/_lib.py:

```python
import ctypes
import os
from ctypes import POINTER, Structure, c_char_p, c_float, c_int, c_long, c_void_p

_HERE = os.path.dirname(os.path.abspath(__file__))
LIB_PATH = os.environ.get('OODGAN_LIB') or os.path.join(_HERE, 'liboodgan_hip.so')

CONV_S1, CONV_T2, CONV_S2 = 0, 1, 2
ACT_NONE, ACT_LRELU, ACT_PRELU = 0, 1, 2

P = c_void_p


ABI_VERSION = 113


class ConvArgs(Structure):
    _fields_ = [
        ('x', P), ('wpk', P), ('in_scale', P), ('in_shift', P), ('out_scale', P), ('bias', P), ('noise', P),
        ('noise_w', P), ('slope', P), ('dotx', P), ('dot_part', P), ('y', P),
        ('B', c_int), ('K', c_int), ('M', c_int), ('Hin', c_int), ('Win', c_int),
        ('in_pitch', c_int), ('out_pitch', c_int), ('in_scale_stride', c_int), ('out_scale_stride', c_int),
        ('noise_batch', c_int), ('mode', c_int), ('act', c_int), ('dot_nparts', c_int), ('in_mul2', P),
        ('x_sform', c_int), ('ys', P), ('ys_scale', P), ('ys_scale_stride', c_int),
        ('rgb_w', P), ('rgb_s', P), ('rgb_y', P), ('rgb_s_stride', c_int), ('rgb_scale', c_float), ('fuse', P), ('dot_actgrad', c_int), ('groups', c_int), ('y_fform', c_int), ('x_fform', c_int), ('dotx_fform', c_int), ('dotx_sform', c_int), ('dotx_scale', P), ('dotx_scale_stride', c_int), ('workspace', P), ('workspace_bytes', c_long), ('ys_vmax', P), ('x_hi_only', c_int),
# ... 8 lines not shown

class ReduceJob(Structure):
    _fields_ = [('part', P), ('out', P), ('B', c_int), ('C', c_int), ('nparts', c_int), ('out_stride', c_int), ('accumulate', c_int),
                ('part2', P), ('scale2', P), ('nparts2', c_int), ('scale2_stride', c_int)]


class DemodBwdJob(Structure):
    _fields_ = [('s', P), ('wsq', P), ('d', P), ('r', P), ('gs', P), ('s_stride', c_int), ('d_stride', c_int), ('gs_stride', c_int),
                ('B', c_int), ('Ci', c_int), ('Co', c_int), ('scale', c_float)]


class DemodFwdJob(Structure):
    _fields_ = [('s', P), ('wsq', P), ('d', P), ('s_stride', c_int), ('d_stride', c_int), ('B', c_int), ('Ci', c_int), ('Co', c_int),
                ('scale', c_float)]


class ScaleCheckJob(Structure):
    _fields_ = [('part', P), ('n', c_long), ('state', P)]


_SIGS = {
    'oodgan_version': (c_int, []),
    'oodgan_last_error': (c_char_p, []),
    'oodgan_device_count': (c_int, []),
    'oodgan_set_tunable': (c_int, [c_char_p, c_long]),
    'oodgan_get_tunable': (c_long, [c_char_p]),
    'oodgan_dispatch_count': (c_long, [c_char_p]),
    'oodgan_dispatch_reset': (c_int, []),
    'oodgan_zero': (c_int, [P, c_long, P]),
    'oodgan_bias_act_fwd': (c_int, [P, P, P, P, P, c_int, c_int, c_long, c_int, c_float, c_float, P]),
    'oodgan_bias_act_bwd': (c_int, [P, P, P, P, c_int, c_int, c_long, c_float, c_float, P]),
    'oodgan_upfirdn2d': (c_int, [P, P, P] + [c_int] * 15 + [P]),
    'oodgan_blur_bias_act': (c_int, [P, P, P] + [c_int] * 9 + [P, P, c_int, P, c_int, P]),
    'oodgan_style_affine_fwd': (c_int, [P, P, P, P, P, c_int, c_int, c_int, c_int, c_float, c_float, P]),
    'oodgan_style_affine_bwd': (c_int, [P, P, P, P, c_int, c_int, c_int, c_int, c_float, P]),
    'oodgan_equal_linear': (c_int, [P, P, P, P, c_int, c_int, c_int, c_float, c_float, c_int, P]),
    'oodgan_equal_linear_grouped': (c_int, [P, P, P, P, c_int, c_int, c_int, c_int, c_float, c_float, c_int, P]),
    'oodgan_pixel_norm': (c_int, [P, P, c_int, c_int, P]),
    'oodgan_weight_sqsum': (c_int, [P, P, c_int, c_int, c_int, P]),
    'oodgan_demod_fwd': (c_int, [P, c_int, P, P, c_int, c_int, c_int, c_int, c_float, P]),
    'oodgan_demod_bwd': (c_int, [P, c_int, P, P, c_int, P, P, c_int, c_int, c_int, c_int, c_float, P]),
    'oodgan_pack_conv3x3': (c_int, [P, P, c_int, c_int, c_float, c_int, c_int, P]),
    'oodgan_conv3x3': (c_int, [POINTER(ConvArgs), P]),
    'oodgan_conv3x3_nparts': (c_int, [c_int, c_int, c_int]),
    'oodgan_pack_conv3x3_f16s_bytes': (c_long, [c_int, c_int, c_int]),
    'oodgan_pack_conv3x3_f16s': (c_int, [P, P, P, c_int, c_int, c_float, c_int, c_int, P]),
    'oodgan_conv3x3_f16s': (c_int, [POINTER(ConvArgs), P, P]),
    'oodgan_conv3x3_f16s_nparts': (c_int, [c_int, c_int, c_int]),
    'oodgan_conv3x3_f16s_nparts2': (c_int, [c_int, c_int, c_int, c_int]),
    'oodgan_conv3x3_s2_fuse_supported': (c_int, [c_int, c_int, c_int, c_int, c_int]),
    'oodgan_conv3x3_s1_ys_supported': (c_int, [c_int, c_int, c_int, c_int, c_int]),
    'oodgan_conv3x3_s2_grouped_supported': (c_int, [c_int, c_int, c_int, c_int, c_int, c_int]),
    'oodgan_conv3x3_s1_actgrad_supported': (c_int, [c_int, c_int, c_int, c_int, c_int]),
    'oodgan_sform_bytes': (c_long, [c_int, c_int, c_int, c_int]),
    'oodgan_sform_phases_bytes': (c_long, [c_int, c_int, c_int, c_int]),
    'oodgan_blurT_to_sform_phases': (c_int, [P, P, P, c_int, P, P, c_int, c_int, c_int, c_int, P]),
    'oodgan_from_sform': (c_int, [P, P, c_int, P, c_int, c_int, c_int, c_int, P]),
    'oodgan_to_sform_phases': (c_int, [P, P, c_int, P, P, c_int, c_int, c_int, c_int, c_int, P]),
    'oodgan_to_sform_phases_padtl': (c_int, [P, P, c_int, P, P, c_int, c_int, c_int, c_int, c_int, P]),
    'oodgan_to_sform': (c_int, [P, P, c_int, P, c_int, P, P, c_int, c_int, c_int, c_int, c_int, P, P]),
    'oodgan_resize_bicubic_ac': (c_int, [P, P, P, c_int, c_int, c_int, c_int, c_int, P]),
    'oodgan_avgpool': (c_int, [P, P, c_int, c_int, c_int, c_int, c_int, P]),
    'oodgan_blur_act_sform': (c_int, [P, P, P, P, P, c_int, P, P, c_int, P, c_int, c_int, c_int, c_int, c_int, c_int, P, P]),
    'oodgan_blur_act_sform_sep': (c_int, [P, P, P, P, P, c_int, P, P, c_int, P, c_int, c_int, c_int, c_int, c_int, c_int, P, c_int, P]),
    'oodgan_blur_act_fform': (c_int, [P, P, P, P, c_int, P, P, c_int, P, c_int, c_int, c_int, c_int, c_int, c_int, P, c_int, P]),
    'oodgan_conv3x3_xf_supported': (c_int, [c_int, c_int, c_int, c_int, c_int]),
    'oodgan_upconv_vblur_supported': (c_int, [c_int, c_int, c_int, c_int, c_int]),
    'oodgan_upconv_vblur_fform': (c_int, [P, P, c_long, P, P, P, c_int, P, P, c_int, P, c_int, P, c_int, P, P, c_int, c_int, c_int, c_int, c_int, P]),
    'oodgan_conv3x3_xf_nparts': (c_int, [c_int, c_int, c_int]),
    'oodgan_conv3x3_tiny_workspace': (c_long, [c_int, c_int, c_int, c_int, c_int, c_int]),

    'oodgan_absmax_scaled': (c_int, [P, P, c_int, P, c_int, c_int, c_long, P]),
    'oodgan_fwd_range_update': (c_int, [P, P, P, c_int, P]),
    'oodgan_fwd_range_plan': (c_int, [P, P, P, P, P, P, P, c_int, c_int, c_int, c_int, c_int, c_int, c_int, P]),
    'oodgan_act_bwd_sform_nparts': (c_int, [c_int, c_int]),
    'oodgan_act_bwd_sform': (c_int, [P, P, P, c_int, P, P, P, P, P, c_int, c_float, P, c_int, P, P, P, P, P, c_int, c_int, c_int, c_int, P]),
    'oodgan_act_bwd_sform_f': (c_int, [P, P, c_int, P, P, P, P, P, c_int, c_float, P, c_int, P, P, P, P, P, c_int, c_int, c_int, c_int, P]),
    'oodgan_from_fform': (c_int, [P, P, c_int, c_int, c_int, c_int, P]),
    'oodgan_act_bwd_blurT_nparts': (c_int, [c_int, c_int]),
    'oodgan_act_bwd_blurT_pre_supported': (c_int, [c_int, c_int]),
    'oodgan_act_bwd_blurT_sform_phases': (c_int, [P, P, P, c_int, P, P, P, P, P, c_int, c_float, P, c_int, P, P, P, P, P, P, c_int, c_int, c_int, c_int, P]),
    'oodgan_act_bwd_blurT_hi_supported': (c_int, [c_int, c_int]),
    'oodgan_conv3x3_s1_xh_supported': (c_int, [c_int, c_int, c_int, c_int, c_int]),
    'oodgan_act_bwd_blurT_sform_phases_hi': (c_int, [P, P, P, c_int, P, P, P, c_int, P, P, P, P, P, c_int, c_int, c_int, c_int, P]),
    'oodgan_absmax_scale_check': (c_int, [P, c_long, P, P, P]),
    'oodgan_reduce_batch': (c_int, [P, c_int, P]),
    'oodgan_demod_bwd_batch': (c_int, [P, c_int, P]),
    'oodgan_demod_fwd_batch': (c_int, [P, c_int, P]),
    'oodgan_absmax_scale_check_batch': (c_int, [P, c_int, P, P]),
    'oodgan_hform_bytes': (c_long, [c_int, c_int, c_int, c_int]),
    'oodgan_to_hform': (c_int, [P, P, c_int, c_int, c_int, c_int, P]),
    'oodgan_from_hform': (c_int, [P, P, c_int, c_int, c_int, c_int, P]),
    'oodgan_modconv_f16_wbytes': (c_long, [c_int, c_int, c_int]),
    'oodgan_modconv_f16_pack': (c_int, [P, P, c_int, c_float, c_int, c_int, P, c_int, c_int, c_int, P]),
    'oodgan_modconv_f16_pack_affine': (c_int, [P, P, c_int, P, P, c_int, c_float, c_int, c_int, P, c_int, c_int, c_int, P]),
    'oodgan_modconv_f16': (c_int, [P, P, P, c_int, P, P, c_int, P, c_int, c_int, c_int, c_int, c_int, P]),
    'oodgan_reduce_parts': (c_int, [P, P, c_long, c_int, c_int, P]),
    'oodgan_reduce_parts_cols': (c_int, [P, P, c_int, c_int, c_int, c_int, c_int, P]),
    'oodgan_torgb_fwd': (c_int, [P, P, P, c_int, P, P, P, P, c_int, c_int, c_int, c_int, c_float, P]),
    'oodgan_rgb_finish': (c_int, [P, P, P, P, P, c_int, c_int, c_int, P]),
    'oodgan_rgb_finish_parts': (c_int, [P, c_int, P, P, P, P, c_int, c_int, c_int, P]),
    'oodgan_torgb_fwd_sform': (c_int, [P, P, P, c_int, P, P, P, P, P, P, c_int, c_int, c_int, c_int, c_int, c_float, P, P]),
    'oodgan_act_bwd_fused': (c_int, [P, P, P, c_int, P, P, P, P, P, c_int, c_float, P, P, P, c_int, c_int, c_long, P]),
    'oodgan_act_bwd_nparts': (c_int, [c_long]),
    'oodgan_feature_modulation': (c_int, [P, P, P, P, c_long, c_int, P]),
    'oodgan_act_bwd_fused_max': (c_int, [P, P, P, c_int, P, P, P, P, P, c_int, c_float, P, P, P, P, P, c_int, c_int, c_int, c_long, P]),
    'oodgan_absmax_scale': (c_int, [P, c_long, P, P]),
    'oodgan_absmax_scale_clear': (c_int, [P, c_long, P, P]),
    'oodgan_mse_fwd_bwd': (c_int, [P, P, P, P, P, c_int, c_long, c_float, P]),
    'oodgan_mse_fwd_bwd_row': (c_int, [P, P, P, P, P, P, c_int, c_int, c_long, c_float, P]),
    'oodgan_conv2d_s1': (c_int, [P, P, P, P, P, P, c_int, c_int, c_int, c_int, c_int, c_int, c_int, c_int, P]),
    'oodgan_add_mask': (c_int, [P, P, P, c_long, P]),
    'oodgan_maxpool3s2_fwd': (c_int, [P, P, P, c_long, c_int, c_int, P]),
    'oodgan_maxpool3s2_bwd': (c_int, [P, P, P, P, P, c_long, c_int, c_int, P]),
    'oodgan_lpips_prep': (c_int, [P, P, c_int, c_int, c_int, c_float, c_float, POINTER(c_float), POINTER(c_float), P]),
    'oodgan_lpips_img_grad': (c_int, [P, P, c_int, c_int, c_int, c_float, c_float, POINTER(c_float), P]),
    'oodgan_lpips_head': (c_int, [P, P, P, P, P, c_int, c_int, c_long, c_float, c_int, P]),
    'oodgan_lpips_head_nparts': (c_int, [c_long]),
    'oodgan_lpips_finish': (c_int, [POINTER(P), POINTER(c_int), POINTER(c_long), c_int, P, P, c_int, c_int, P]),
    'oodgan_plan_create': (P, []),
    'oodgan_plan_destroy': (c_int, [P]),
    'oodgan_plan_record_begin': (c_int, [P]),
    'oodgan_plan_record_end': (c_long, [P]),
    'oodgan_plan_size': (c_long, [P]),
    'oodgan_plan_run': (c_int, [P, c_int]),
    'oodgan_plan_set_null_launch': (c_int, [c_int]),
    'oodgan_mse_nparts': (c_int, [c_long]),
    'oodgan_composite_mse_fwd_bwd': (c_int, [P, P, P, P, P, P, P, c_int, c_int, c_long, c_int, c_float, P]),
    'oodgan_composite_mse_fwd_bwd_row': (c_int, [P, P, P, P, P, P, P, P, c_int, c_int, c_int, c_long, c_int, c_float, P]),
    'oodgan_scale_by_plane': (c_int, [P, P, c_int, c_int, c_long, P]),
    'oodgan_loss_weight_from_alpha': (c_int, [P, P, c_long, c_int, P]),
    'oodgan_ssim_nparts': (c_int, [c_int, c_int, c_int]),
    'oodgan_ssim_loss_fwd_bwd': (c_int, [P, P, P, P, P, c_int, c_int, c_int, c_int, c_float, P]),
    'oodgan_ssim_loss_fwd_bwd_row': (c_int, [P, P, P, P, P, P, c_int, c_int, c_int, c_int, c_int, c_float, P]),
    'oodgan_robust_loss_fwd_bwd': (c_int, [P, P, P, P, P, P, P, c_int, c_int, c_long, c_int, c_float, c_int, c_float, P]),
    'oodgan_robust_loss_fwd_bwd_row': (c_int, [P, P, P, P, P, P, P, P, c_int, c_int, c_int, c_long, c_int, c_float, c_int, c_float, P]),
    'oodgan_area_pool_fwd': (c_int, [P, P, P, c_int, c_int, c_int, c_int, P]),
    'oodgan_area_pool_bwd_add': (c_int, [P, P, c_int, c_int, c_int, c_int, P]),
    'oodgan_adam_step': (c_int, [P, P, P, P, c_long, c_float, c_float, c_float, c_float, c_int, P]),
    'oodgan_adam_step_dev': (c_int, [P, P, P, P, c_long, c_float, c_float, c_float, c_float, P, P]),
    'oodgan_adam_step_dev_sched': (c_int, [P, P, P, P, c_long, c_float, c_float, c_float, c_float, P, c_int, c_float, c_float, P]),
    'oodgan_latent_noise': (c_int, [P, P, P, P, c_int, c_long, c_long, c_int, c_float, c_float, P]),
    'oodgan_latent_prior_fwd_bwd': (c_int, [P, P, P, P, c_int, c_long, c_int, c_float, P]),
    'oodgan_latent_prior_fwd_bwd_row': (c_int, [P, P, P, P, P, c_int, c_int, c_long, c_int, c_float, P]),
}

_lib = None


def lib():
    global _lib
    if _lib is None:
        if not os.path.exists(LIB_PATH):
            raise RuntimeError(
                f'{LIB_PATH} not found: build it with `python __graft_entry__.py` (hipcc --offload-arch=gfx950); '
                'there is no CPU or PyTorch fallback for the hot path')
        h = ctypes.CDLL(LIB_PATH)
        for name, (res, args) in _SIGS.items():
            fn = getattr(h, name, None)
            if fn is None:
                continue
            fn.restype = res
            fn.argtypes = args
        if h.oodgan_version() != ABI_VERSION:
            raise RuntimeError(f'{LIB_PATH} has ABI version {h.oodgan_version()}, this host layer needs exactly {ABI_VERSION} (the argument structs must match): rebuild the library')
        _lib = h
# ... 39 lines not shown
```

ood-gan-inversion_amd/oodgan/engine.py:

```python
import math
import numbers
import re

import os

import torch

from . import ops
from ._lib import ACT_LRELU, ACT_NONE, CONV_S1, CONV_S2, CONV_T2
from .synth import generator_channels, make_kernel


_Cols = ops.Cols


class _Layer:
    __slots__ = ('name', 'kind', 'cin', 'cout', 'res', 'lat', 'row', 'drow', 'wpk', 'wpk_bwd', 'wsq', 'w_rgb',
                 'bias', 'noise_w', 'scale', 'noise_idx', 'src', 'sidx', 'wpk_vb')


def _pad_channels_to_16(state, prefix, log_size, ch):
    up16 = lambda c: (c + 15) // 16 * 16
    chp = {r: up16(c) for r, c in ch.items()}
    out = dict(state)
# ... 52 lines not shown
        if any(c < 1 for c in used):
            raise ValueError(f'channel counts {used} (narrow={narrow}, channel_multiplier={channel_multiplier})')
        self.padded = any(c % 16 for c in used)
        self.real_channels = dict(ch)
        if self.padded:
            state, _ = _pad_channels_to_16(state, prefix, self.log_size, ch)
        g = lambda k: state[prefix + k].detach().float().contiguous()
        dev = g('input.input').device
        if dev.type != 'cuda':
            raise RuntimeError('GeneratorEngine needs its parameters on a ROCm device (no CPU fallback)')
        self.device = dev
        self.const_input = g('input.input')
        def family(pattern, taps, what):
            pat = re.compile('^' + re.escape(prefix) + pattern + r'\.kernel$')
            held = [v.detach().float().cpu() for k, v in state.items() if pat.match(k)]
            k4 = held[0] if held else make_kernel(tuple(taps)) * 4.0
            if tuple(k4.shape) != (4, 4):
                raise NotImplementedError(f'{what} kernel of shape {tuple(k4.shape)}: the fused producers are built for four taps (every shipped config: [1,3,3,1])')
            if any(h.shape != k4.shape or not torch.equal(h, k4) for h in held):
                raise NotImplementedError(f'the {what} kernels of the state differ between layers')
            return k4.contiguous()

        k4 = family(r'convs\.\d+\.conv\.blur', blur_kernel, 'Blur')
        self.k4x4 = k4.to(dev)
        self.k4x4_flip = torch.flip(self.k4x4, [0, 1]).contiguous()
        self.k4x4_rank1 = bool(torch.linalg.matrix_rank(k4.double()) == 1)
        self.k_up = family(r'to_rgbs\.\d+\.upsample', upsample_kernel, 'Upsample').to(dev)
        self.k_up_flip = torch.flip(self.k_up, [0, 1]).contiguous()
        layers = []

        up16 = lambda c: (c + 15) // 16 * 16

        def styled(name, cin, cout, res, lat, up, nidx):
            L = _Layer()
            L.name, L.kind, L.cin, L.cout, L.res, L.lat, L.noise_idx = name, ('up' if up else 'conv'), up16(cin), up16(cout), res, lat, nidx
            w = g(f'{name}.conv.weight')[0]
            L.scale = 1.0 / math.sqrt(cin * 9)
            L.wpk = ops.pack_conv3x3(w, L.scale, transpose=False, flip=False, precision=self.precision)
            L.wpk_bwd = ops.pack_conv3x3(w, L.scale, transpose=True, flip=not up, precision=self.precision) if with_backward else None
            if L.wpk_bwd is not None:
                L.wpk_bwd.x_hi_only = self.grad_hi_only
            L.wsq = ops.weight_sqsum(w)
            L.wpk_vb = None
            L.bias = g(f'{name}.activate.bias')
            L.noise_w = g(f'{name}.noise.weight')
            layers.append(L)
            return L

        def rgb(name, cin, res, lat):
            L = _Layer()
            L.name, L.kind, L.cin, L.cout, L.res, L.lat = name, 'rgb', up16(cin), 3, res, lat
            L.w_rgb = g(f'{name}.conv.weight').reshape(3, up16(cin)).contiguous()
            L.bias = g(f'{name}.bias').reshape(3).contiguous()
            L.scale = 1.0 / math.sqrt(up16(cin))
            layers.append(L)
            return L

        styled('conv1', ch[4], ch[4], 4, 0, False, 0)
        rgb('to_rgb1', ch[4], 4, 1)
        cin, i = ch[4], 1
        for j in range(self.log_size - 2):
            res = 2 ** (j + 3)
            cout = ch[res]
            styled(f'convs.{2 * j}', cin, cout, res, i, True, 2 * j + 1)
            styled(f'convs.{2 * j + 1}', cout, cout, res, i + 1, False, 2 * j + 2)
            rgb(f'to_rgbs.{j}', cout, res, i + 2)
            cin, i = cout, i + 2
        self.layers = layers
        self.fused_bwd = True
        self.bwd_state, self.bwd_flag = {}, None
        styled = [L for L in layers if L.kind != 'rgb']
        self.layers_styled_last = styled[-1]
        self.fused_fwd = True
        self.next_conv = {a.name: b for a, b in zip(styled[:-1], styled[1:]) if a.kind == 'up' and b.kind == 'conv'}
        self.rgb_next_up = {a.name: b for a, b in zip(layers[:-1], layers[1:]) if a.kind == 'rgb' and b.kind == 'up'}
        self.conv_next_rgb = {a.name: b for a, b in zip(layers[:-1], layers[1:]) if a.kind == 'conv' and b.kind == 'rgb'}
        self.by_name = {L.name: L for L in layers}
        self.fuse_act_bwd = True
        self.hi_records = os.environ.get('OODGAN_HI_RECORDS', '1') != '0'
        self.fused_rgb = True
        self.fuse_x = True
        self.fuse_up = True
        self.save_sform_only = os.environ.get('OODGAN_SAVE_SFORM_ONLY', '1') != '0'
        self.fuse_conv_rgb_64 = True
        self.sform_only_max_res = None
        self.fuse_conv_rgb = os.environ.get('OODGAN_FUSE_CONV_RGB', '1') != '0'
        self.plain_one_pass = os.environ.get('OODGAN_PLAIN_ONE_PASS', '1') != '0'
        Lup = next((a for a, b in zip(styled[:-1], styled[1:]) if a.kind == 'up' and b is styled[-1]), None)
        if (Lup is not None and self.precision == 'f16s' and self.sform and with_backward and Lup.cout % 32 == 0 and Lup.cin % 16 == 0
                and Lup.cout <= 32 and size >= 64):
            Lup.wpk_vb = ops.pack_upconv_vblur(g(f'{Lup.name}.conv.weight')[0], Lup.scale, self.k4x4)
        ops.xf_supported(1, 32, 32, 8, 32)
        self.batched_tail = True
        src = 'input'
        for L in layers:
            L.src = src
            if L.kind != 'rgb':
                src = L.name
        rows, drows, wl, bl, rl = 0, 0, [], [], []
        lat_start = [0] * (self.n_latent + 1)
        row_layer, drow_layer, sidx = [], [], 0
        for L in layers:
            L.row = rows
            wl.append(g(f'{L.name}.conv.modulation.weight'))
            bl.append(g(f'{L.name}.conv.modulation.bias'))
            rl += [L.lat] * L.cin
            rows += L.cin
            lat_start[L.lat + 1] = rows
            if L.kind != 'rgb':
                L.drow = drows
                drows += L.cout
                L.sidx = sidx
                row_layer += [sidx] * L.cin
                drow_layer += [sidx] * L.cout
                sidx += 1
            else:
                L.sidx = -1
                row_layer += [-1] * L.cin
        for l in range(1, self.n_latent + 1):
            lat_start[l] = max(lat_start[l], lat_start[l - 1])
        self.R, self.DR = rows, drows
        self.wcat = torch.cat(wl, 0).contiguous()
        self.bcat = torch.cat(bl, 0).contiguous()
        self.row_lat = torch.tensor(rl, dtype=torch.int32, device=dev)
        self.lat_start = torch.tensor(lat_start, dtype=torch.int32, device=dev)
        self.row_layer = torch.tensor(row_layer, dtype=torch.int32, device=dev)
        self.drow_layer = torch.tensor(drow_layer, dtype=torch.int32, device=dev)
        self.n_styled = sidx
        self.fwd_range = None
        self.carry_range = True
        self.stored_noises = [g(f'noises.noise_{k}') for k in range(self.num_layers)] if (prefix + 'noises.noise_0') in state else None
        self.saved = None

    def clone_shared(self):
        import copy
        e = copy.copy(self)
        e.saved = None
        e.bwd_state, e.bwd_flag = {}, None
        e.fwd_range = None
        e._ranges = {}
        return e

    def reset_fwd_state(self, B=None):
        ranges = self.__dict__.get('_ranges', {})
        todo = list(ranges.values()) if B is None else [r for r in (ranges.get(B),) if r is not None]
        if self.fwd_range is not None and (B is None or self.fwd_range.B == B) and not any(r is self.fwd_range for r in todo):
            todo.append(self.fwd_range)
        for r in todo:
            r.valid = False
            r.flag.zero_()
            r.vm.zero_()

    def fwd_range_violated(self):
        return self.fwd_range is not None and self.fwd_range.violated()

    def _range(self, B):
        if self.fwd_range is None or self.fwd_range.B != B:
            ranges = self.__dict__.setdefault('_ranges', {})
            r = ranges.get(B)
            if r is None:
                r = ranges[B] = ops.FwdRange(self.n_styled, B, self.R, self.DR, self.row_layer, self.drow_layer, self.device)
            self.fwd_range = r
        return self.fwd_range

    def reset_bwd_state(self):
        self.bwd_state = {}
# ... 90 lines not shown
                    elif pending is not None:
                        xs, pending = pending, None
                    else:
                        xs = to_s(L, out)
                    Lr = self.conv_next_rgb.get(L.name) if self.fused_rgb else None
                    if Lr is not None and 16 < L.cin <= 32 and 16 < L.cout <= 32:
                        ff = (save and carry and self.fused_bwd and L is self.layers_styled_last and L.cout == 32
                              and self.bwd_state.get(L.name) is not None and not return_features)
                        out, rgb_partial = ops.conv3x3(xs, L.wpk, L.cout, CONV_S1, out_scale=d, bias=L.bias, noise=nz,
                                                       noise_weight=L.noise_w, act=ACT_LRELU, rgb=(Lr.w_rgb, _Cols(s_all, Lr.row, Lr.cin)),
                                                       y_fform=ff or xf_in, in_scale=_Cols(s_use, L.row, L.cin) if xf_in else None)
                    else:
                        Lu = self.rgb_next_up.get(Lr.name) if (Lr is not None and carry) else None
                        Hc, Wc = xs.shape[2], xs.shape[3]
                        if (Lu is not None and self.fuse_conv_rgb and not xf_in and L.cout % 16 == 0 and Hc * Wc > (4095 if self.fuse_conv_rgb_64 else 4096) and Wc % 4 == 0
                                and ops.s1_ys_supported(B, L.cin, L.cout, Hc, Wc)):
                            pending = ops.sform_scratch(B, L.cout, Hc, Wc, self.device, tag=4)
                            sform_only = (save and self.save_sform_only and self.fused_bwd and self.fuse_act_bwd
                                          and (self.sform_only_max_res is None or Hc <= self.sform_only_max_res)
                                          and self.bwd_state.get(L.name) is not None and self.bwd_state.get(Lu.name) is not None
                                          and ops.s2_fuse_supported(B, Lu.cout, Lu.cin, 2 * Hc + 1, 2 * Wc + 1))
                            keep = (save and not sform_only) or return_features or post_hook is not None
                            out, rgb_partial = ops.conv3x3(xs, L.wpk, L.cout, CONV_S1, out_scale=d, bias=L.bias, noise=nz, noise_weight=L.noise_w,
                                                           act=ACT_LRELU, rgb=(Lr.w_rgb, _Cols(s_all, Lr.row, Lr.cin)), ys=pending,
                                                           ys_scale=_Cols(s_use, Lu.row, Lu.cin), vmax=rng.vm[Lu.sidx], want_y=keep)
                            if not keep:
                                out = ops.SFormSaved(pending, _Cols(s_use, Lu.row, Lu.cin))
                        else:
                            out = ops.conv3x3(xs, L.wpk, L.cout, CONV_S1, out_scale=d, bias=L.bias, noise=nz,
                                              noise_weight=L.noise_w, act=ACT_LRELU)
                    del xs
                else:
                    out = ops.conv3x3(out, L.wpk, L.cout, CONV_S1, in_scale=s, out_scale=d, bias=L.bias, noise=nz,
                                      noise_weight=L.noise_w, act=ACT_LRELU)
            else:
                Hi = out.shape[2]
                Ln = self.next_conv.get(L.name)
                ff_tail = (self.sform and carry and self.fused_fwd and Ln is not None and save and self.fuse_x and self.fused_bwd and self.fused_rgb
                           and Ln is self.layers_styled_last and not return_features
                           and self.bwd_state.get(Ln.name) is not None and self.bwd_state.get(L.name) is not None
                           and ops.xf_supported(B, Ln.cin, Ln.cout, 2 * Hi, 2 * Hi))
                one_pass = ff_tail and self.fuse_up and L.wpk_vb is not None and ops.upconv_vblur_supported(B, L.cin, L.cout, Hi, Hi)
                plain_tail = (self.sform and not save and not one_pass and self.plain_one_pass and self.fuse_up and self.fuse_x
                              and self.fused_rgb and Ln is not None and Ln is self.layers_styled_last and L.wpk_vb is not None
                              and Ln.name in self.conv_next_rgb and 16 < Ln.cin <= 32 and 16 < Ln.cout <= 32
                              and not (cond_layers is not None and L.lat in cond_layers)
                              and not (features_in is not None and Ln.lat < len(features_in) and features_in[Ln.lat] is not None)
                              and ops.upconv_vblur_supported(B, L.cin, L.cout, Hi, Hi) and ops.xf_supported(B, Ln.cin, Ln.cout, 2 * Hi, 2 * Hi))
                z = None
                if self.sform:
                    if pending is not None:
                        xs, pending = pending, None
                    else:
                        xs = to_s(L, out)
                    if one_pass:
                        out = ops.upconv_vblur_fform(xs, L.wpk_vb, out_scale=d, bias=L.bias, noise=nz, noise_weight=L.noise_w, act=True,
                                                     ys_scale=_Cols(s_use, Ln.row, Ln.cin), vmax=rng.vm[Ln.sidx])
                    elif plain_tail:
                        out = ops.upconv_vblur_fform(xs, L.wpk_vb, out_scale=d, bias=L.bias, noise=nz, noise_weight=L.noise_w, act=True,
                                                     ys_scale=_Cols(s_use if carry else s_all, Ln.row, Ln.cin), vmax=rng.vm[Ln.sidx])
                        if not carry:
                            rng.update_exact(Ln.sidx)
                            rng.plan(s_all, d_all, Ln.row, Ln.cin, Ln.drow, Ln.cout)
                        one_pass = True
                    else:
                        z = ops.conv3x3(xs, L.wpk, L.cout, CONV_T2, out_scale=d)
                    del xs
                else:
                    z = ops.conv3x3(out, L.wpk, L.cout, CONV_T2, in_scale=s, out_scale=d)
                H2 = 2 * Hi + 1
                lat_idx = L.lat
                if one_pass:
                    pass
                elif cond_hook is not None and cond_layers is not None and lat_idx in cond_layers:
                    raw = ops.blur_bias_act(z, self.k4x4, (1, 1), act=False, in_hw=(H2, H2), in_pitch=z.shape[3])
                    cond = cond_hook(cond_layers.index(lat_idx), raw, latent[:, lat_idx], nz, L.noise_w)
                    out = ops.bias_noise_act(cond, L.bias, nz, L.noise_w)
                elif carry and self.fused_fwd and L.name in self.next_conv:
                    if ff_tail:
                        out = ops.blur_act_fform(z, self.k4x4, Hi, Hi, L.bias, nz, L.noise_w, act=True,
                                                 ys_scale=_Cols(s_use, Ln.row, Ln.cin), vmax=rng.vm[Ln.sidx], rank_one=self.k4x4_rank1)
                    else:
                        pending = ops.sform_scratch(B, L.cout, 2 * Hi, 2 * Hi, self.device, tag=2)
                        out = ops.blur_act_sform(z, self.k4x4, Hi, Hi, L.bias, nz, L.noise_w, act=True, ys=pending,
                                                 ys_scale=_Cols(s_use, Ln.row, Ln.cin), vmax=rng.vm[Ln.sidx], rank_one=self.k4x4_rank1)
                else:
                    out = ops.blur_bias_act(z, self.k4x4, (1, 1), L.bias, nz, L.noise_w, act=True, in_hw=(H2, H2),
                                            in_pitch=z.shape[3])
                del z
                if post_hook is not None and cond_layers is not None and lat_idx in cond_layers:
                    out = post_hook(cond_layers.index(lat_idx), out)
                    pending = None
            acts[L.name] = out
        if rng is not None:
            if carry:
                rng.finish()
            else:
                rng.valid = True
        if save:
            self.saved = dict(acts=acts, s_all=s_all, d_all=d_all, noises=noises, B=B, serial=self._fwd_serial)
        if return_features:
            feat = out.to_nchw() if isinstance(out, ops.FForm) else out
            return skip, (feat[:, :self.real_channels[self.size]].contiguous() if self.padded else feat)
        return skip

    def _demod(self, L, s_all, d_all):
        from ._lib import lib, check
        import ctypes
        B = s_all.shape[0]
        check(lib().oodgan_demod_fwd(ctypes.c_void_p(s_all.data_ptr() + 4 * L.row), self.R, ctypes.c_void_p(L.wsq.data_ptr()),
                                     ctypes.c_void_p(d_all.data_ptr() + 4 * L.drow), self.DR, B, L.cin, L.cout, L.scale,
                                     ops._stream()), 'demod_fwd')

    def _hi_records(self, B, L, Hd, Rg):
        return bool(self.grad_hi_only and self.hi_records and Rg is None and ops.blurT_hi_supported(Hd, Hd)
                    and ops.s2_fuse_supported(B, L.cout, L.cin, 2 * Hd + 1, 2 * Hd + 1))

    def backward(self, gimg, grad_scale=1.0, carry_scale=False):
        from ._lib import lib, check
        import ctypes
        sv = self.saved
        if sv is None:
            raise RuntimeError('backward() without forward(save=True)')
        if sv.get('serial') != getattr(self, '_fwd_serial', None):
            raise RuntimeError('backward(): another forward of this engine ran after forward(save=True) — the saved activations (pooled S-form / F-form '
                               'buffers, scales of the range state) may have been overwritten; call backward() right after the forward it belongs to')
        acts, s_all, d_all, noises, B = sv['acts'], sv['s_all'], sv['d_all'], sv['noises'], sv['B']
        gs_all = ops.zeros(B, self.R, device=self.device)
        gskip = {self.size: gimg.contiguous()}
        r = self.size
        while r > 4:
            gskip[r // 2] = ops.upfirdn2d(gskip[r], self.k_up_flip, up=1, down=2, pad=(1, 1))
            r //= 2
        g_feat = None
        prev_rgb = None
        fused_in = None
        fused_pre = None
        jobs = ops.BwdJobs() if (carry_scale and self.fused_bwd and self.sform and self.batched_tail) else None
        for L in reversed(self.layers):
            if L.kind == 'rgb':
                prev_rgb = L
                continue
            out, x_in, nz = acts[L.name], acts[L.src], noises[L.noise_idx]
            fused_ok = carry_scale and self.fused_bwd and self.bwd_state.get(L.name) is not None
            xf_bwd = (fused_ok and g_feat is None and L.kind == 'conv' and isinstance(out, ops.FForm) and isinstance(x_in, ops.FForm)
                      and prev_rgb is not None and self.fuse_x)
            if isinstance(out, ops.FForm) and not (fused_ok and (g_feat is None or fused_pre is not None)):
                out = out.to_nchw()
            if isinstance(out, ops.SFormSaved) and fused_in is None:
                out = out.to_nchw()
            if isinstance(x_in, ops.FForm) and not xf_bwd:
                x_in = x_in.to_nchw()
            s = _Cols(s_all, L.row, L.cin)
            d = _Cols(d_all, L.drow, L.cout)
            Hd = x_in.shape[2]
            carry = carry_scale and self.fused_bwd and self.sform and (L.kind == 'conv' or Hd >= 4)
            st = self.bwd_state.get(L.name) if carry else None
            Rg, prev_rgb = prev_rgb, None
            rgb_kw = {} if Rg is None else dict(g_rgb=gskip[L.res], w_rgb=Rg.w_rgb, s_rgb=_Cols(s_all, Rg.row, Rg.cin))
            if st is not None and fused_in is not None:
                gin, rsum, tsum, part_m = fused_in.dst, fused_in.r, None, fused_in.part_m
                fused_in = None
                mul2, g_pre = st, None
            elif st is not None and xf_bwd:
                gin, rsum, tsum, part_m = None, None, None, None
                mul2, g_pre = st, None
            elif st is not None:
                t_into = None if Rg is None else _Cols(gs_all, Rg.row, Rg.cin)
                if L.kind == 'conv':
                    gin = ops.sform_scratch(B, L.cout, out.shape[2], out.shape[3], self.device)
                    rsum, tsum, part_m = ops.act_bwd_producer(out, g_feat, nz, L.noise_w, L.bias, d, st, gin, t_into=t_into, jobs=jobs, **rgb_kw)
                elif fused_pre is not None:
                    gin = ops.sform_phases_scratch(B, L.cout, Hd, Hd, self.device)
                    rsum, tsum, part_m = ops.act_bwd_producer(None, g_feat, nz, L.noise_w, L.bias, d, st, gin, blur_kernel=self.k4x4_flip,
                                                              jobs=jobs, dot_of=fused_pre, hi_only=self._hi_records(B, L, Hd, Rg))
                    fused_pre = None
                else:
                    gin = ops.sform_phases_scratch(B, L.cout, Hd, Hd, self.device)
                    rsum, tsum, part_m = ops.act_bwd_producer(out, g_feat, nz, L.noise_w, L.bias, d, st, gin,
                                                              blur_kernel=self.k4x4_flip, t_into=t_into, jobs=jobs,
                                                              hi_only=self._hi_records(B, L, Hd, Rg), **rgb_kw)
                mul2, g_pre = st, None
            else:
                if Rg is not None:
                    g_pre, rsum, tsum, mul2 = ops.act_bwd_fused(out, g_feat, nz, L.noise_w, L.bias, gskip[L.res], Rg.w_rgb,
                                                                _Cols(s_all, Rg.row, Rg.cin), want_scale=True, dscale=d)
                else:
                    g_pre, rsum, tsum, mul2 = ops.act_bwd_fused(out, g_feat, nz, L.noise_w, L.bias, want_scale=True, dscale=d)
                if carry:
                    self.bwd_state[L.name] = mul2
                    if self.bwd_flag is None:
                        self.bwd_flag = torch.zeros(1, dtype=torch.int32, device=self.device)
            if Rg is not None and tsum is not None:
                gs_all[:, Rg.row:Rg.row + Rg.cin] = tsum
            deferred = st is not None and jobs is not None
            xa = None
            if st is not None and xf_bwd:
                xa = ops.ActBwdX(nz, L.noise_w, L.bias, d, st, gskip[L.res], Rg.w_rgb, _Cols(s_all, Rg.row, Rg.cin),
                                 t_into=_Cols(gs_all, Rg.row, Rg.cin))
                pre = None
                Lp = self.by_name.get(L.src)
                if (Lp is not None and Lp.kind == 'up' and self.fuse_act_bwd and self.bwd_state.get(L.src) is not None
                        and ops.s1_actgrad_supported(B, L.cout, L.cin, out.shape[2], out.shape[3])):
                    pre = ops.DotActGrad()
                dx, dot = ops.conv3x3(out, L.wpk_bwd, L.cin, CONV_S1, out_scale=s, dotx=x_in, in_mul2=mul2,
                                      dot_into=_Cols(gs_all, L.row, L.cin), jobs=jobs, dot_actgrad=pre, xf_act=xa)
                rsum, part_m = xa.r, xa.part_m
                fused_in, fused_pre = None, pre
            if deferred:
                jobs.add_demod(_Cols(s_all, L.row, L.cin), L.wsq, _Cols(d_all, L.drow, L.cout), rsum, _Cols(gs_all, L.row, L.cin), B, L.cin,
                               L.cout, L.scale)
            else:
                check(lib().oodgan_demod_bwd(ctypes.c_void_p(s_all.data_ptr() + 4 * L.row), self.R, ctypes.c_void_p(L.wsq.data_ptr()),
                                             ctypes.c_void_p(d_all.data_ptr() + 4 * L.drow), self.DR, ctypes.c_void_p(rsum.data_ptr()),
                                             ctypes.c_void_p(gs_all.data_ptr() + 4 * L.row), self.R, B, L.cin, L.cout, L.scale,
                                             ops._stream()), 'demod_bwd')
            if xa is not None:
                if deferred:
                    jobs.add_check(part_m, st)
                else:
                    ops.absmax_scale_check(part_m, st, self.bwd_flag)
            elif st is not None:
                fz = None
                Lp = self.by_name.get(L.src)
                stp = self.bwd_state.get(L.src) if (L.kind == 'up' and Lp is not None and self.fuse_act_bwd) else None
                if stp is not None and ops.s2_fuse_supported(B, L.cout, L.cin, 2 * Hd + 1, 2 * Hd + 1):
                    Rp = self.conv_next_rgb[Lp.name]
                    hi = bool(self.grad_hi_only and self.hi_records and ops.s1_xh_supported(B, Lp.cout, Lp.cin, Hd, Hd))
                    fz = ops.ActBwdFusion((ops.sform_hi_scratch if hi else ops.sform_scratch)(B, Lp.cout, Hd, Hd, self.device), noises[Lp.noise_idx],
                                          Lp.noise_w, Lp.bias, _Cols(d_all, Lp.drow, Lp.cout), stp, g_rgb=gskip[Lp.res], w_rgb=Rp.w_rgb,
                                          s_rgb=_Cols(s_all, Rp.row, Rp.cin), t_into=_Cols(gs_all, Rp.row, Rp.cin), hi_only=hi)
                pre = None
# ... 494 lines not shown
```

ood-gan-inversion_amd/oodgan/ops.py:

```python
import ctypes
import os
import math

import torch

from . import _lib
from ._lib import ACT_LRELU, ACT_NONE, ACT_PRELU, CONV_S1, CONV_S2, CONV_T2, ConvArgs, check

SQRT2 = 2 ** 0.5


def _p(t):
    return None if t is None else ctypes.c_void_p(t.data_ptr())


_RAW_STREAM = getattr(torch._C, '_cuda_getCurrentRawStream', None)
_DEV_INDEX = None


def _stream_handle():
    global _DEV_INDEX
    if _RAW_STREAM is None:
        return torch.cuda.current_stream().cuda_stream
    if _DEV_INDEX is None:
# ... 279 lines not shown
        return self.data.data_ptr()

    @property
    def shape(self):
        return (self.B, self.C, 2 * self.H + 1, 2 * self.W + 1)


def to_sform_phases(x, H, W, scale=None, mul2=None, out=None, in_pitch=0, pad_tl=False):
    x = _dev(x)
    B, C = x.shape[0], x.shape[1]
    if out is None:
        out = SFormPhases(B, C, H, W, x.device)
    out.hi_only = False
    fn = _lib.lib().oodgan_to_sform_phases_padtl if pad_tl else _lib.lib().oodgan_to_sform_phases
    check(fn(_p(x), _p(_opt(scale, 'scale')), 0 if scale is None else scale.shape[1], _p(mul2), _p(out), B, C, H, W, in_pitch, _stream()),
          'to_sform_phases')
    return out


def blurT_to_sform_phases(g, kernel, scale=None, mul2=None, out=None):
    g = _dev(g)
    B, C = g.shape[0], g.shape[1]
    H, W = g.shape[2] // 2, g.shape[3] // 2
    if out is None:
        out = SFormPhases(B, C, H, W, g.device)
    out.hi_only = False
    check(_lib.lib().oodgan_blurT_to_sform_phases(_p(g), _p(_dev(kernel)), _p(_opt(scale, 'scale')),
                                                  0 if scale is None else scale.shape[1], _p(mul2), _p(out), B, C, H, W,
                                                  _stream()), 'blurT_to_sform_phases')
    return out


_SFORM_POOL = {}


def sform_phases_scratch(B, C, H, W, device):
    key = ('ph', B, C, H, W, str(device), _stream_handle())
    buf = _SFORM_POOL.get(key)
    if buf is None:
        buf = _SFORM_POOL[key] = SFormPhases(B, C, H, W, device)
    return buf


_WS_POOL = {}
USE_TINY = True


def conv_workspace(nbytes, device):
    key = (nbytes, str(device), _stream_handle())
    buf = _WS_POOL.get(key)
    if buf is None:
        buf = _WS_POOL[key] = torch.empty(nbytes // 4, device=device, dtype=torch.int32)
    return buf


def drop_stream_scratch(stream_handle):
    for pool in (_SFORM_POOL, _WS_POOL):
        for key in [k for k in pool if k[-1] == stream_handle]:
            del pool[key]
    for key in [k for k in _VMAX_POOL if k[1] == stream_handle]:
        del _VMAX_POOL[key]


def sform_scratch(B, C, H, W, device, tag=0):
    key = (B, C, H, W, str(device), tag, _stream_handle())
    buf = _SFORM_POOL.get(key)
    if buf is None:
        buf = _SFORM_POOL[key] = SForm(B, C, H, W, device)
    return buf


def to_sform(x, scale=None, mul2=None, out=None, in_hw=None, in_pitch=0, vmax=None, shift=None):
    x = _dev(x)
    B, C = x.shape[0], x.shape[1]
    H, W = in_hw if in_hw is not None else (x.shape[2], x.shape[3])
    if out is None:
        out = SForm(B, C, H, W, x.device)
    check(_lib.lib().oodgan_to_sform(_p(x), _p(_opt(scale, 'scale')), 0 if scale is None else scale.shape[1],
                                     _p(_opt(shift, 'shift')), 0 if shift is None else shift.shape[1], _p(mul2), _p(out),
                                     B, C, H, W, in_pitch, _p(vmax), _stream()), 'to_sform')
    return out


def blur_act_sform(z, kernel, H, W, bias=None, noise=None, noise_weight=None, act=True, ys=None, ys_scale=None, vmax=None, rank_one=False):
    z = _dev(z)
    B, C = z.shape[0], z.shape[1]
    y = torch.empty(B, C, 2 * H, 2 * W, device=z.device, dtype=torch.float32)
    nz = _opt(noise, 'noise')
    check(_lib.lib().oodgan_blur_act_sform_sep(_p(z), _p(_dev(kernel, 'kernel')), _p(y), _p(ys), _p(_opt(ys_scale, 'ys_scale')),
                                               0 if ys_scale is None else ys_scale.shape[1], _p(_opt(bias, 'bias')), _p(nz),
                                               1 if nz is None else nz.shape[0], _p(_opt(noise_weight, 'nw')),
                                               ACT_LRELU if act else ACT_NONE, B, C, H, W, z.shape[3], _p(vmax), 1 if rank_one else 0,
                                               _stream()), 'blur_act_sform')
    return y


def blur_act_fform(z, kernel, H, W, bias=None, noise=None, noise_weight=None, act=True, ys_scale=None, vmax=None, rank_one=False):
    z = _dev(z)
    B, C = z.shape[0], z.shape[1]
    y = torch.empty(B, C, 2 * H, 2 * W, device=z.device, dtype=torch.float32)
    nz = _opt(noise, 'noise')
    check(_lib.lib().oodgan_blur_act_fform(_p(z), _p(_dev(kernel, 'kernel')), _p(y), _p(_opt(ys_scale, 'ys_scale')),
                                           0 if ys_scale is None else ys_scale.shape[1], _p(_opt(bias, 'bias')), _p(nz),
                                           1 if nz is None else nz.shape[0], _p(_opt(noise_weight, 'nw')),
                                           ACT_LRELU if act else ACT_NONE, B, C, H, W, z.shape[3], _p(vmax), 1 if rank_one else 0, _stream()),
          'blur_act_fform')
    return FForm(y)


def xf_supported(B, K, M, H, W):
    return bool(_lib.lib().oodgan_conv3x3_xf_supported(B, K, M, H, W))


VMAX_SLOTS = 64


def absmax_mul2(x):
    x = _dev(x)
    B, C = x.shape[0], x.shape[1]
    key = (str(x.device), _stream_handle(), B)
    vm = _VMAX_POOL.get(key)
    if vm is None:
        vm = _VMAX_POOL[key] = torch.zeros(B * VMAX_SLOTS, device=x.device, dtype=torch.int32)
    mul2 = torch.empty(2, device=x.device, dtype=torch.float32)
    L = _lib.lib()
    check(L.oodgan_absmax_scaled(_p(x), None, 0, _p(vm), B, C, x.numel() // (B * C), _stream()), 'absmax_scaled')
    check(L.oodgan_absmax_scale_clear(_p(vm), vm.numel(), _p(mul2), _stream()), 'absmax_scale_clear')
    return mul2


_VMAX_POOL = {}


class FwdRange:

    def __init__(self, n_layers, B, R, DR, row_layer, drow_layer, device):
        self.L, self.B, self.R, self.DR = n_layers, B, R, DR
        self.q = torch.ones(n_layers, B, device=device, dtype=torch.float32)
        self.vm = torch.zeros(n_layers, B, VMAX_SLOTS, device=device, dtype=torch.int32)
        self.flag = torch.zeros(1, device=device, dtype=torch.int32)
        self.s_sc = torch.empty(B, R, device=device, dtype=torch.float32)
        self.d_sc = torch.empty(B, DR, device=device, dtype=torch.float32)
        self.row_layer, self.drow_layer = row_layer, drow_layer
        self.valid = False

    def plan(self, s_all, d_all, row0=0, nrows=None, drow0=0, ndrows=None):
        nrows = self.R if nrows is None else nrows
        ndrows = self.DR if ndrows is None else ndrows
        check(_lib.lib().oodgan_fwd_range_plan(_p(s_all), _p(d_all), _p(self.row_layer), _p(self.drow_layer), _p(self.q), _p(self.s_sc),
                                               _p(self.d_sc), self.B, self.R, self.DR, row0, nrows, drow0, ndrows, _stream()),
              'fwd_range_plan')

    def measure(self, l, x, s):
        x = _dev(x)
        B, C = x.shape[0], x.shape[1]
        check(_lib.lib().oodgan_absmax_scaled(_p(x), _p(s), s.shape[1], _p(self.vm[l]), B, C, x.numel() // (B * C), _stream()),
              'absmax_scaled')
        check(_lib.lib().oodgan_fwd_range_update(_p(self.vm[l]), _p(self.q[l]), None, B, _stream()), 'fwd_range_update')

    def update_exact(self, l):
        check(_lib.lib().oodgan_fwd_range_update(_p(self.vm[l]), _p(self.q[l]), None, self.B, _stream()), 'fwd_range_update')

    def finish(self):
        check(_lib.lib().oodgan_fwd_range_update(_p(self.vm), _p(self.q), _p(self.flag), self.L * self.B, _stream()), 'fwd_range_update')

    def violated(self):
        return int(self.flag.item()) != 0


class BwdJobs:

    def __init__(self):
        self.reduce, self.reduce_acc, self.demod, self.check, self.keep = [], [], [], [], []

    def add_reduce(self, part, out_ptr_obj, B, C, nparts, out_stride, accumulate, second=None):
        (self.reduce_acc if accumulate else self.reduce).append(_reduce_job(part, out_ptr_obj, B, C, nparts, out_stride, accumulate, second))
        self.keep += [part, out_ptr_obj, second]
# ... 259 lines not shown
    M = wvb.M
    y = torch.empty(B, M, 2 * H, 2 * W, device=xs.data.device, dtype=torch.float32)
    nz = _opt(noise, 'noise')
    check(_lib.lib().oodgan_upconv_vblur_fform(_p(xs), _p(wvb.data), wvb.wset_bytes, _p(wvb.unscale4), _p(wvb.kh),
                                               _p(_opt(out_scale, 'out_scale')), 0 if out_scale is None else out_scale.shape[1],
                                               _p(_opt(bias, 'bias')), _p(nz), 1 if nz is None else nz.shape[0],
                                               _p(_opt(noise_weight, 'nw')), ACT_LRELU if act else ACT_NONE,
                                               _p(_opt(ys_scale, 'ys_scale')), 0 if ys_scale is None else ys_scale.shape[1], _p(vmax),
                                               _p(y), B, K, M, H, W, _stream()), 'upconv_vblur_fform')
    return FForm(y)


def conv3x3(x, wpk, M, mode=CONV_S1, in_scale=None, in_shift=None, out_scale=None, bias=None, noise=None,
            noise_weight=None, act=ACT_NONE, slope=None, dotx=None, in_hw=None, in_pitch=0, out=None, out_pitch=0,
            in_mul2=None, ys=None, ys_scale=None, want_y=True, dot_into=None, rgb=None, jobs=None, fuse=None, dot_actgrad=None,
            groups=1, y_fform=False, xf_act=None, tiny_max=8, vmax=None):
    sform_in = isinstance(x, (SForm, SFormPhases))
    fform_in = isinstance(x, FForm)
    if fform_in:
        assert mode == CONV_S1 and wpk.precision == 'f16s'
        y_fform = xf_act is None
    elif not sform_in:
        x = _dev(x)
    B, K = x.shape[0], x.shape[1] // max(1, groups)
    H, W = in_hw if in_hw is not None else (x.shape[2], x.shape[3])
    if mode == CONV_S1:
        oh, ow = H, W
    elif mode == CONV_T2:
        oh, ow = 2 * H + 1, 2 * W + 1
        if out_pitch == 0:
            out_pitch = (ow + 3) // 4 * 4
    else:
        oh, ow = (H - 1) // 2, (W - 1) // 2
    pitch = out_pitch if out_pitch else ow
    if out is None and want_y:
        out = torch.empty(B, M, oh, pitch, device=x.data.device if (sform_in or fform_in) else x.device, dtype=torch.float32)
    a = ConvArgs()
    a.x, a.wpk, a.y = _p(x), _p(wpk), _p(out)
    a.in_scale, a.in_shift, a.out_scale = _p(_opt(in_scale, 'in_scale')), _p(_opt(in_shift, 'in_shift')), _p(_opt(out_scale, 'out_scale'))
    a.bias, a.noise, a.noise_w, a.slope = _p(_opt(bias, 'bias')), _p(_opt(noise, 'noise')), _p(_opt(noise_weight, 'nw')), _p(_opt(slope, 'slope'))
    a.B, a.K, a.M, a.Hin, a.Win = B, K, M, H, W
    a.in_pitch, a.out_pitch = in_pitch, out_pitch
    a.in_scale_stride = in_scale.shape[1] if in_scale is not None else 0
    a.out_scale_stride = out_scale.shape[1] if out_scale is not None else 0
    a.noise_batch = noise.shape[0] if noise is not None else 1
    a.mode, a.act = mode, act
    a.in_mul2 = _p(in_mul2)
    a.x_sform = 1 if sform_in else 0
    a.x_fform = (2 if xf_act is not None else 1) if fform_in else 0
    ws = None
    if sform_in and USE_TINY and wpk.precision == 'f16s' and mode in (CONV_S1, CONV_S2) and min(oh, ow) <= tiny_max:
        nb = _lib.lib().oodgan_conv3x3_tiny_workspace(mode, B, K, M, H, W)
        if nb > 0:
            ws = conv_workspace(nb, x.data.device)
            a.workspace, a.workspace_bytes = _p(ws), nb
    a.groups = int(groups)
    a.x_hi_only = 1 if (wpk.x_hi_only and dotx is not None) else 0
    if isinstance(x, (SForm, SFormPhases)) and x.hi_only:
        assert a.x_hi_only == 1, 'hi-only input records need the two-instruction input-gradient conv (precision f16s-g2, dotx)'
        a.x_hi_only = 2
    a.y_fform = 1 if y_fform else 0
    a.ys, a.ys_scale = _p(ys), _p(_opt(ys_scale, 'ys_scale'))
    a.ys_vmax = _p(vmax)
    rgb_y = None
    if rgb is not None:
        w_rgb, s_rgb = rgb
        nrgb = 1 if M <= 32 else (M + 63) // 64
        rgb_y = torch.empty(*((B, 3, oh, ow) if nrgb == 1 else (nrgb, B, 3, oh, ow)), device=x.data.device if sform_in or fform_in else x.device,
                            dtype=torch.float32)
        a.rgb_w, a.rgb_s, a.rgb_y = _p(_dev(w_rgb, 'w_rgb').reshape(3, M)), _p(_dev(s_rgb, 's_rgb')), _p(rgb_y)
        a.rgb_s_stride, a.rgb_scale = s_rgb.shape[1], 1.0 / math.sqrt(M)
    a.ys_scale_stride = ys_scale.shape[1] if ys_scale is not None else 0
    fz = None
    if fuse is not None:
        fz = fuse.struct(B, M, oh, ow)
        a.fuse = ctypes.cast(ctypes.pointer(fz), ctypes.c_void_p)
    if xf_act is not None:
        fz = xf_act.struct(B, K, H, W)
        a.fuse = ctypes.cast(ctypes.pointer(fz), ctypes.c_void_p)
    part = None
    if dotx is not None:
        dot_f = isinstance(dotx, FForm)
        dot_s = isinstance(dotx, SFormSaved)
        if dot_s and fuse is None:
            dotx, dot_s = dotx.to_nchw(), False
        dx_ = dotx.data if dot_f else (dotx.sform.data if dot_s else _dev(dotx, 'dotx'))
        a.dotx_fform = 1 if dot_f else 0
        if dot_s:
            a.dotx_sform, a.dotx_scale, a.dotx_scale_stride = 1, _p(dotx.scale), dotx.scale.shape[1]
        if fform_in:
            npart = _lib.lib().oodgan_conv3x3_xf_nparts(B, H, W)
        elif wpk.precision == 'f16s':
            npart = _lib.lib().oodgan_conv3x3_f16s_nparts2(mode, H, W, 1 if sform_in else 0)
        else:
            npart = _lib.lib().oodgan_conv3x3_nparts(mode, H, W)
        part = torch.empty(B, M, npart, device=dx_.device, dtype=torch.float32)
        a.dotx, a.dot_part, a.dot_nparts = _p(dx_), _p(part), npart
        if dot_actgrad is not None:
            a.dot_actgrad = 1
            dot_actgrad.dot_part, dot_actgrad.scale = part, out_scale
    if wpk.precision == 'f16s':
        check(_lib.lib().oodgan_conv3x3_f16s(ctypes.byref(a), _p(wpk.unscale), _stream()), 'conv3x3_f16s')
    else:
        check(_lib.lib().oodgan_conv3x3(ctypes.byref(a), _stream()), 'conv3x3')
    if fuse is not None:
        fuse.finish(part, a.dot_nparts, jobs)
    if xf_act is not None:
        xf_act.finish(jobs)
    if dotx is not None:
        if dot_into is not None:
            if jobs is not None:
                jobs.add_reduce(part, dot_into, B, M, a.dot_nparts, dot_into.shape[1], True)
            else:
                _reduce_into(part, B, M, a.dot_nparts, dot_into, True)
            return out, None
        dot = torch.empty(B, M, device=dx_.device, dtype=torch.float32)
        check(_lib.lib().oodgan_reduce_parts(_p(part), _p(dot), B * M, a.dot_nparts, 0, _stream()), 'reduce_parts')
        return out, dot
    if y_fform:
        out = FForm(out)
    if rgb is not None:
        return out, rgb_y
    return out


def s2_fuse_supported(B, K, M, Hin, Win):
    return bool(_lib.lib().oodgan_conv3x3_s2_fuse_supported(B, K, M, Hin, Win))


def tiny_workspace_bytes(mode, B, K, M, Hin, Win):
    return int(_lib.lib().oodgan_conv3x3_tiny_workspace(mode, B, K, M, Hin, Win)) if USE_TINY else 0


def s1_xh_supported(B, K, M, H, W):
    return bool(_lib.lib().oodgan_conv3x3_s1_xh_supported(B, K, M, H, W))


def sform_hi_scratch(B, C, H, W, device):
    buf = sform_scratch(B, C, H, W, device, tag='hi')
    buf.hi_only = True
    return buf


def s1_ys_supported(B, K, M, H, W):
    return bool(_lib.lib().oodgan_conv3x3_s1_ys_supported(B, K, M, H, W))


def s2_grouped_supported(B, K, M, groups, Hin, Win):
    return bool(_lib.lib().oodgan_conv3x3_s2_grouped_supported(B, K, M, groups, Hin, Win))


def s1_actgrad_supported(B, K, M, H, W):
    return bool(_lib.lib().oodgan_conv3x3_s1_actgrad_supported(B, K, M, H, W))


class DotActGrad:
    __slots__ = ('dot_part', 'scale')

    def __init__(self):
        self.dot_part = self.scale = None


class ActBwdFusion:

    def __init__(self, dst, noise, noise_weight, bias, dscale, mul2, g_rgb=None, w_rgb=None, s_rgb=None, t_into=None, hi_only=False):
        self.hi_only = bool(hi_only)
        self.dst, self.noise, self.noise_weight, self.bias, self.dscale, self.mul2 = dst, _opt(noise, 'noise'), _opt(noise_weight, 'nw'), _opt(bias, 'bias'), dscale, mul2
        self.g_rgb, self.w_rgb, self.s_rgb, self.t_into = _opt(g_rgb, 'g_rgb'), w_rgb, s_rgb, t_into
        self.r = self.t = self.part_m = None

    def struct(self, B, M, H, W):
        dev = self.dst.data.device
        ntile = ((H + 7) // 8) * ((W + 31) // 32)
        self.B, self.M = B, M
        self.part_r = torch.empty(B, M, ntile, device=dev, dtype=torch.float32)
        self.part_t = torch.empty(B, M, ntile, device=dev, dtype=torch.float32) if self.g_rgb is not None else None
        self.part_m = zeros(B * ntile * ((M + 63) // 64) * 8, device=dev)
        z = _lib.ActBwdFuse()
        z.g_rgb, z.noise, z.noise_w, z.bias = _p(self.g_rgb), _p(self.noise), _p(self.noise_weight), _p(self.bias)
        self._w = None if self.w_rgb is None else _dev(self.w_rgb).reshape(3, M)
        z.w_rgb, z.s_rgb = _p(self._w), _p(self.s_rgb)
        z.s_rgb_stride = 0 if self.s_rgb is None else self.s_rgb.shape[1]
        z.noise_batch = 1 if self.noise is None else self.noise.shape[0]
        z.dscale, z.dscale_stride, z.mul2, z.ys = _p(self.dscale), self.dscale.shape[1], _p(self.mul2), _p(self.dst)
        z.part_r, z.part_t, z.part_max = _p(self.part_r), _p(self.part_t), _p(self.part_m)
        z.rgb_scale, z.nmax = 1.0 / math.sqrt(M), self.part_m.numel()
        z.ys_hi_only = 1 if self.hi_only else 0
        assert self.dst.hi_only == self.hi_only, 'a hi-only S-form scratch is dedicated to hi-only records'
        return z

    def finish(self, dot_part, nparts, jobs):
        B, M = self.B, self.M
        if jobs is not None:
            self.r = torch.empty(B, M, device=self.part_r.device, dtype=torch.float32)
            jobs.add_reduce(self.part_r, self.r, B, M, nparts, M, False)
            if self.part_t is not None:
                jobs.add_reduce(self.part_t, self.t_into, B, M, nparts, self.t_into.shape[1], False)
            return
        self.r = _reduce_parts(self.part_r, B * M, nparts)
        if self.part_t is not None:
            if self.t_into is not None:
                _reduce_into(self.part_t, B, M, nparts, self.t_into, False)
            else:
                self.t = _reduce_parts(self.part_t, B * M, nparts)


class ActBwdX:

    def __init__(self, noise, noise_weight, bias, dscale, mul2, g_rgb, w_rgb, s_rgb, t_into=None):
        self.noise, self.noise_weight, self.bias, self.dscale, self.mul2 = _opt(noise, 'noise'), _opt(noise_weight, 'nw'), _opt(bias, 'bias'), dscale, mul2
        self.g_rgb, self.w_rgb, self.s_rgb, self.t_into = _dev(g_rgb, 'g_rgb'), w_rgb, s_rgb, t_into
        self.r = self.t = self.part_m = None

    def struct(self, B, C, H, W):
        dev = self.g_rgb.device
        self.B, self.C = B, C
        self.nparts = _lib.lib().oodgan_conv3x3_xf_nparts(B, H, W)
        self.part_r = torch.empty(B, C, self.nparts, device=dev, dtype=torch.float32)
        self.part_t = torch.empty(B, C, self.nparts, device=dev, dtype=torch.float32)
        self.part_m = torch.empty(B * ((C + 15) // 16) * self.nparts, device=dev, dtype=torch.float32)
# ... 338 lines not shown
```

Measured before the change: 7.808.

## Skip saving fp32 up-layer activations; read S-form records as dotx in stride-1 backward conv

For upsampling layers in the forward pass, the blur+activation producer can now write only the hi/lo f16 S-form records, with no fp32 NCHW output. The stride-1 8-wave backward conv gains a DS template path that reads the dot operand straight from those S-form records, undoing the per-channel scale through a reciprocal and a sign mask. This removes one full-resolution fp32 write and its later re-read, plus the to_nchw conversion. The ys store in the YS path is also reworked to use permlane16_swap for full 16-byte stores. In exchange there are more kernel instantiations and a dot operand reconstructed from the hi+lo split, which may differ slightly in precision.

```diff
diff --git a/include/oodgan.h b/include/oodgan.h
--- a/include/oodgan.h
+++ b/include/oodgan.h
@@ -206,6 +206,7 @@
                                       float* part_r, float* part_t, float* part_max, int B, int C, int H, int W, void* stream);
 int oodgan_act_bwd_blurT_hi_supported(int H, int W);
 int oodgan_conv3x3_s1_xh_supported(int B, int K, int M, int H, int W);
+int oodgan_conv3x3_s1_dotx_sform_supported(int B, int K, int M, int H, int W);
 int oodgan_act_bwd_blurT_sform_phases_hi(const float* g_feat, const float* out, const float* noise, int noise_batch, const float* noise_w,
                                          const float* bias, const float* dscale, int dscale_stride, const float* mul2, const float* kernel,
                                          void* out_phases, float* part_r, float* part_max, int B, int C, int H, int W, void* stream);
diff --git a/ood-gan-inversion_amd/csrc/common.hpp b/ood-gan-inversion_amd/csrc/common.hpp
--- a/ood-gan-inversion_amd/csrc/common.hpp
+++ b/ood-gan-inversion_amd/csrc/common.hpp
@@ -37,7 +37,8 @@
        OODGAN_DC_COMPOSITE_MSE,
        OODGAN_DC_SSIM,
        OODGAN_DC_ROBUST,
-       OODGAN_DC_AREA_POOL, OODGAN_DC_COUNT };
+       OODGAN_DC_AREA_POOL,
+       OODGAN_DC_S1BIG_DOTXS, OODGAN_DC_COUNT };
 void count_dispatch(int id);
 
 bool bound_device_ok(const char* what);
diff --git a/ood-gan-inversion_amd/csrc/conv_f16s.hip b/ood-gan-inversion_amd/csrc/conv_f16s.hip
--- a/ood-gan-inversion_amd/csrc/conv_f16s.hip
+++ b/ood-gan-inversion_amd/csrc/conv_f16s.hip
@@ -417,6 +417,14 @@
     return (H > 8 && W > 8 && !s1_strip_eligible(a) && s1_big_eligible(a)) ? 1 : 0;
 }
 
+extern "C" int oodgan_conv3x3_s1_dotx_sform_supported(int B, int K, int M, int H, int W) {
+    oodgan_conv_args a = {};
+    a.mode = OODGAN_CONV_S1; a.x_sform = 1; a.B = B; a.K = K; a.M = M; a.Hin = H; a.Win = W;
+    a.y = reinterpret_cast<float*>(1);
+    a.dotx = reinterpret_cast<const float*>(1);
+    return (H > 8 && W > 8 && !s1_strip_eligible(a) && s1_big_eligible(a)) ? 1 : 0;
+}
+
 extern "C" int oodgan_conv3x3_s1_ys_supported(int B, int K, int M, int H, int W) {
     oodgan_conv_args a = {};
     a.mode = OODGAN_CONV_S1; a.x_sform = 1; a.B = B; a.K = K; a.M = M; a.Hin = H; a.Win = W;
@@ -448,10 +456,11 @@
                    "conv3x3_f16s: the F-form output exists only in the strip kernel (mode S1, S-form input, 16 < K,M <= 32)");
     OODGAN_REQUIRE(!a.dot_actgrad || (a.mode == OODGAN_CONV_S1 && a.x_sform && a.dotx && (s1_strip_eligible(a) || s1_big_eligible(a))),
                    "conv3x3_f16s: dot_actgrad exists only in the strip / 8-wave kernels of mode S1 (oodgan_conv3x3_s1_actgrad_supported)");
-    OODGAN_REQUIRE(!a.dotx_sform || (a.mode == OODGAN_CONV_S2 && a.x_sform && a.fuse && a.dotx && a.dotx_scale && a.dotx_scale_stride >= a.M &&
-                                     !tiny_eligible(a) && s2_big_eligible(a)),
-                   "conv3x3_f16s: dotx_sform needs mode S2, a phase-split S-form input, `fuse`, dotx, dotx_scale and a shape of the 8-wave kernel "
-                   "(oodgan_conv3x3_s2_fuse_supported)");
+    OODGAN_REQUIRE(!a.dotx_sform || (a.x_sform && a.dotx && a.dotx_scale && a.dotx_scale_stride >= a.M && !tiny_eligible(a) &&
+                                     ((a.mode == OODGAN_CONV_S2 && a.fuse && s2_big_eligible(a)) ||
+                                      (a.mode == OODGAN_CONV_S1 && !s1_strip_eligible(a) && s1_big_eligible(a)))),
+                   "conv3x3_f16s: dotx_sform needs an S-form input, dotx, dotx_scale and a shape of an 8-wave kernel: mode S2 with `fuse` "
+                   "(oodgan_conv3x3_s2_fuse_supported) or mode S1 (oodgan_conv3x3_s1_dotx_sform_supported)");
     OODGAN_REQUIRE(a.ys_vmax == nullptr || (a.ys != nullptr && a.mode == OODGAN_CONV_S1 && a.x_sform && !tiny_eligible(a) && !s1_strip_eligible(a) && s1_big_eligible(a)),
                    "conv3x3_f16s: ys_vmax only with ys from the 8-wave stride-1 kernel (oodgan_conv3x3_s1_ys_supported)");
     OODGAN_REQUIRE(a.x_hi_only != 2 || (a.x_sform && a.dotx && !tiny_eligible(a) &&
diff --git a/ood-gan-inversion_amd/csrc/conv_f16s_big.hip b/ood-gan-inversion_amd/csrc/conv_f16s_big.hip
--- a/ood-gan-inversion_amd/csrc/conv_f16s_big.hip
+++ b/ood-gan-inversion_amd/csrc/conv_f16s_big.hip
@@ -44,7 +44,7 @@
 __device__ long g_s1big_stamp_n = 0;
 #endif
 
-template <bool DOT, bool PRE, bool YS = false, bool G2 = false>
+template <bool DOT, bool PRE, bool YS = false, bool G2 = false, bool DS = false>
 __global__ __launch_bounds__(512) void conv_f16s_s1big_kernel(const BigConv p, const uint4* __restrict__ wpk16) {
     constexpr int NW = 8, NT = 2;
     extern __shared__ __attribute__((aligned(16))) unsigned char smem[];
@@ -198,6 +198,7 @@
         const int m = m0 + tid;
         cst_o = a.out_scale ? a.out_scale[(long)b * a.out_scale_stride + m] : 1.f;
         if (!DOT && a.bias) cst_b = a.bias[m];
+        if (DS) cst_b = 1.f / a.dotx_scale[(long)b * a.dotx_scale_stride + m];
         if (!DOT && a.act == OODGAN_ACT_PRELU) cst_s = a.slope[m];
         if (YS && a.rgb_y) {
             const float sv = a.rgb_scale * a.rgb_s[(long)b * a.rgb_s_stride + m];
@@ -216,6 +217,7 @@
         float* cst = reinterpret_cast<float*>(smem + BG_CST);
         cst[tid] = cst_o;
         if (!DOT) { cst[64 + tid] = cst_b; cst[128 + tid] = cst_s; }
+        if (DS) cst[64 + tid] = cst_b;
         if (YS) {
             float* rw = reinterpret_cast<float*>(smem + BG_RGBW);
             rw[tid] = rgb_c0; rw[64 + tid] = rgb_c1; rw[128 + tid] = rgb_c2;
@@ -279,6 +281,11 @@
         dsum[q] = 0.f;
     }
     const bool mfull = m0 + 64 <= M;
+    unsigned dsgn[16];
+    if (DS) {
+#pragma unroll
+        for (int q = 0; q < 16; ++q) dsgn[q] = __float_as_uint(cst[64 + 16 * (q >> 2) + 4 * g + (q & 3)]) & 0x80000000u;
+    }
     float ysc[16], ysmax = 0.f;
     if (YS) {
 #pragma unroll
@@ -294,9 +301,29 @@
         float nz = 0.f;
         if (has_nz) nz = nw * reinterpret_cast<const float*>(smem + BG_NZ)[wave * 64 + (n >> 1) * 32 + 16 * (n & 1) + n16];
         unsigned char* yr = reinterpret_cast<unsigned char*>(a.y) + ((long)b * M * p.out_plane + (long)py * a.out_pitch + px) * 4;
-        const unsigned char* dr = DOT ? reinterpret_cast<const unsigned char*>(a.dotx) + ((long)b * M * H * W + (long)py * W + px) * 4 : nullptr;
+        const unsigned char* dr = (DOT && !DS) ? reinterpret_cast<const unsigned char*>(a.dotx) + ((long)b * M * H * W + (long)py * W + px) * 4 : nullptr;
         float o[16], dv[16];
-        if (DOT) {
+        if (DOT && DS) {
+            const unsigned char* rb = reinterpret_cast<const unsigned char*>(a.dotx) +
+                                      sform_unit(p.yd, b, 0, min(py, H - 1), min(px, W - 1), ((g & 1) << 1) | (g >> 1)) * 16;
+            const unsigned okm = ok ? 0xFFFFFFFFu : 0u;
+            uint4 u[4];
+#pragma unroll
+            for (int mt = 0; mt < 4; ++mt) u[mt] = *reinterpret_cast<const uint4*>(rb + (long)min((m0 >> 4) + mt, p.yd.KC - 1) * (p.yd.plane * 16));
+#pragma unroll
+            for (int mt = 0; mt < 4; ++mt) {
+                const auto t0 = __builtin_amdgcn_permlane16_swap(u[mt].x, u[mt].z, false, false);
+                const auto t1 = __builtin_amdgcn_permlane16_swap(u[mt].y, u[mt].w, false, false);
+                unsigned w0 = t0[0] & okm, w1 = t0[1] & okm, w2 = t1[0] & okm, w3 = t1[1] & okm;
+                asm volatile("" : "+v"(w0), "+v"(w1), "+v"(w2), "+v"(w3));
+                const oodgan_half2v h0 = __builtin_bit_cast(oodgan_half2v, w0), l0 = __builtin_bit_cast(oodgan_half2v, w1);
+                const oodgan_half2v h1 = __builtin_bit_cast(oodgan_half2v, w2), l1 = __builtin_bit_cast(oodgan_half2v, w3);
+                dv[4 * mt] = (float)h0[0] + (float)l0[0];
+                dv[4 * mt + 1] = (float)h0[1] + (float)l0[1];
+                dv[4 * mt + 2] = (float)h1[0] + (float)l1[0];
+                dv[4 * mt + 3] = (float)h1[1] + (float)l1[1];
+            }
+        } else if (DOT) {
 #pragma unroll
             for (int q = 0; q < 16; ++q) dv[q] = 0.f;
             if (ok) {
@@ -316,7 +343,7 @@
             o[q] = v * osc[q];
             if (DOT) {
                 dsum[q] += (v * us) * dv[q];
-                if (PRE) o[q] *= dv[q] > 0.f ? kSqrt2 : 0.2f * kSqrt2;
+                if (PRE) o[q] *= (DS ? __uint_as_float(__float_as_uint(dv[q]) ^ dsgn[q]) : dv[q]) > 0.f ? kSqrt2 : 0.2f * kSqrt2;
             } else {
                 o[q] += nz + bia[q];
                 if (a.act == OODGAN_ACT_LRELU) o[q] = (o[q] > 0.f ? o[q] : 0.2f * o[q]) * kSqrt2;
@@ -333,21 +360,25 @@
                     if (moff[q] != 0xFFFFFFFFu) *reinterpret_cast<float*>(yr + moff[q]) = o[q];
             }
         }
-        if (YS && !DOT && ok) {
+        if (YS && !DOT) {
+            const unsigned yl = __builtin_amdgcn_mbcnt_hi(~0u, __builtin_amdgcn_mbcnt_lo(~0u, 0u));
+            const int yslot = (int)(((yl >> 3) & 2u) | (yl >> 5));
+            float nmax = 0.f;
 #pragma unroll
             for (int mt = 0; mt < 4; ++mt) {
                 if (m0 + 16 * mt < M) {
                     const float v0 = o[4 * mt] * ysc[4 * mt], v1 = o[4 * mt + 1] * ysc[4 * mt + 1], v2 = o[4 * mt + 2] * ysc[4 * mt + 2],
                                 v3 = o[4 * mt + 3] * ysc[4 * mt + 3];
-                    ysmax = fmaxf(fmaxf(ysmax, fmaxf(fabsf(v0), fabsf(v1))), fmaxf(fabsf(v2), fabsf(v3)));
+                    nmax = fmaxf(fmaxf(nmax, fmaxf(fabsf(v0), fabsf(v1))), fmaxf(fabsf(v2), fabsf(v3)));
                     uint2 hi, lo;
                     split_pair(v0, v1, hi.x, lo.x);
                     split_pair(v2, v3, hi.y, lo.y);
-                    unsigned char* rec = reinterpret_cast<unsigned char*>(a.ys) + sform_unit(p.yd, b, (m0 >> 4) + mt, py, px, g >> 1) * 16 + (g & 1) * 8;
-                    *reinterpret_cast<uint2*>(rec) = hi;
-                    *reinterpret_cast<uint2*>(rec + 32) = lo;
+                    const auto s0 = __builtin_amdgcn_permlane16_swap(hi.x, lo.x, false, false);
+                    const auto s1 = __builtin_amdgcn_permlane16_swap(hi.y, lo.y, false, false);
+                    if (ok) reinterpret_cast<uint4*>(a.ys)[sform_unit(p.yd, b, (m0 >> 4) + mt, py, px, yslot)] = make_uint4(s0[0], s1[0], s0[1], s1[1]);
                 }
             }
+            if (ok) ysmax = fmaxf(ysmax, nmax);
         }
         if (YS && !DOT && a.rgb_y) {
             const float* rw = reinterpret_cast<const float*>(smem + BG_RGBW);
@@ -370,6 +401,7 @@
 #pragma unroll
         for (int q = 0; q < 16; ++q) {
             float v = dsum[q];
+            if (DS) v *= cst[64 + 16 * (q >> 2) + 4 * g + (q & 3)];
             v += dpp_take<0xB1, 0xF>(v);
             v += dpp_take<0x4E, 0xF>(v);
             v += dpp_take<0x141, 0xF>(v);
@@ -431,7 +463,11 @@
                         (void)hipFuncSetAttribute(reinterpret_cast<const void*>(&conv_f16s_s1big_kernel<false, false>), hipFuncAttributeMaxDynamicSharedMemorySize, BG_SMEM16),
                         (void)hipFuncSetAttribute(reinterpret_cast<const void*>(&conv_f16s_s1big_kernel<false, false, true>), hipFuncAttributeMaxDynamicSharedMemorySize, BG_SMEM16),
                         (void)hipFuncSetAttribute(reinterpret_cast<const void*>(&conv_f16s_s1big_kernel<true, false, false, true>), hipFuncAttributeMaxDynamicSharedMemorySize, BG_SMEM16),
-                        (void)hipFuncSetAttribute(reinterpret_cast<const void*>(&conv_f16s_s1big_kernel<true, true, false, true>), hipFuncAttributeMaxDynamicSharedMemorySize, BG_SMEM16), true);
+                        (void)hipFuncSetAttribute(reinterpret_cast<const void*>(&conv_f16s_s1big_kernel<true, true, false, true>), hipFuncAttributeMaxDynamicSharedMemorySize, BG_SMEM16),
+                        (void)hipFuncSetAttribute(reinterpret_cast<const void*>(&conv_f16s_s1big_kernel<true, false, false, false, true>), hipFuncAttributeMaxDynamicSharedMemorySize, BG_SMEM16),
+                        (void)hipFuncSetAttribute(reinterpret_cast<const void*>(&conv_f16s_s1big_kernel<true, true, false, false, true>), hipFuncAttributeMaxDynamicSharedMemorySize, BG_SMEM16),
+                        (void)hipFuncSetAttribute(reinterpret_cast<const void*>(&conv_f16s_s1big_kernel<true, false, false, true, true>), hipFuncAttributeMaxDynamicSharedMemorySize, BG_SMEM16),
+                        (void)hipFuncSetAttribute(reinterpret_cast<const void*>(&conv_f16s_s1big_kernel<true, true, false, true, true>), hipFuncAttributeMaxDynamicSharedMemorySize, BG_SMEM16), true);
     (void)once;
     const uint4* w16 = reinterpret_cast<const uint4*>(wpk16);
     OODGAN_REQUIRE(!a.dot_actgrad || a.dotx, "conv3x3 big: dot_actgrad without dotx");
@@ -439,7 +475,14 @@
     OODGAN_REQUIRE(a.x_hi_only != 2 || g2, "conv3x3 big: hi-only input records (x_hi_only = 2) need dotx (the two-instruction instances)");
     if (g2) count_dispatch(OODGAN_DC_S1BIG_G2);
     if (g2 && a.x_hi_only == 2) count_dispatch(OODGAN_DC_S1BIG_XH);
-    if (a.dot_actgrad && g2) hipLaunchKernelGGL((conv_f16s_s1big_kernel<true, true, false, true>), dim3((unsigned)total), dim3(512), BG_SMEM16, st, p, w16);
+    const bool ds = a.dotx_sform != 0;
+    OODGAN_REQUIRE(!ds || (a.dotx && a.dotx_scale && a.dotx_scale_stride >= a.M), "conv3x3 big: dotx_sform needs dotx and dotx_scale");
+    if (ds) count_dispatch(OODGAN_DC_S1BIG_DOTXS);
+    if (ds && a.dot_actgrad && g2) hipLaunchKernelGGL((conv_f16s_s1big_kernel<true, true, false, true, true>), dim3((unsigned)total), dim3(512), BG_SMEM16, st, p, w16);
+    else if (ds && g2) hipLaunchKernelGGL((conv_f16s_s1big_kernel<true, false, false, true, true>), dim3((unsigned)total), dim3(512), BG_SMEM16, st, p, w16);
+    else if (ds && a.dot_actgrad) hipLaunchKernelGGL((conv_f16s_s1big_kernel<true, true, false, false, true>), dim3((unsigned)total), dim3(512), BG_SMEM16, st, p, w16);
+    else if (ds) hipLaunchKernelGGL((conv_f16s_s1big_kernel<true, false, false, false, true>), dim3((unsigned)total), dim3(512), BG_SMEM16, st, p, w16);
+    else if (a.dot_actgrad && g2) hipLaunchKernelGGL((conv_f16s_s1big_kernel<true, true, false, true>), dim3((unsigned)total), dim3(512), BG_SMEM16, st, p, w16);
     else if (g2) hipLaunchKernelGGL((conv_f16s_s1big_kernel<true, false, false, true>), dim3((unsigned)total), dim3(512), BG_SMEM16, st, p, w16);
     else if (a.dot_actgrad) hipLaunchKernelGGL((conv_f16s_s1big_kernel<true, true>), dim3((unsigned)total), dim3(512), BG_SMEM16, st, p, w16);
     else if (a.dotx) hipLaunchKernelGGL((conv_f16s_s1big_kernel<true, false>), dim3((unsigned)total), dim3(512), BG_SMEM16, st, p, w16);
diff --git a/ood-gan-inversion_amd/csrc/fwd_producers.hip b/ood-gan-inversion_amd/csrc/fwd_producers.hip
--- a/ood-gan-inversion_amd/csrc/fwd_producers.hip
+++ b/ood-gan-inversion_amd/csrc/fwd_producers.hip
@@ -158,7 +158,7 @@
             float* cell = &lst[cc * LS_CH + (pos >> 6) * LS_ROW + (pos & 63)];
             float t = *cell + nz + cb[0][cc];
             if (a.act == OODGAN_ACT_LRELU) t = (t > 0.f ? t : 0.2f * t) * kSqrt2;
-            if (!a.y_fform && kc * 16 + cc < a.C) yp[(long)cc * HWo] = t;
+            if (!a.y_fform && a.y != nullptr && kc * 16 + cc < a.C) yp[(long)cc * HWo] = t;
             const float v = t * cb[1][cc];
             vm = fmaxf(vm, fabsf(v));
             *cell = a.y_fform ? t : v;
@@ -309,7 +309,7 @@
         }
         float (*gb)[GP] = gat[Y & 1];
         if constexpr (SF) {
-            if (FULL || yok) *reinterpret_cast<float4*>(yplane + (long)Y * Wo + gx) = make_float4(t[0], t[1], t[2], t[3]);
+            if ((FULL || yok) && a.y != nullptr) *reinterpret_cast<float4*>(yplane + (long)Y * Wo + gx) = make_float4(t[0], t[1], t[2], t[3]);
             *reinterpret_cast<float4*>(&gb[ch][(4 * q) ^ sw]) = make_float4(t[0] * ysc, t[1] * ysc, t[2] * ysc, t[3] * ysc);
             __syncthreads();
             if (FULL || pok) {
@@ -349,7 +349,7 @@
                            int ys_scale_stride, const float* bias, const float* noise, int noise_batch,
                            const float* noise_w, int act, int B, int C, int H, int W, int in_pitch, unsigned* vmax,
                            int y_fform, int rank_one, void* stream) {
-    OODGAN_REQUIRE(z && kernel && y && B > 0 && C > 0 && H > 0 && W > 0, "blur_act_sform: bad args");
+    OODGAN_REQUIRE(z && kernel && (y || (ys && !y_fform)) && B > 0 && C > 0 && H > 0 && W > 0, "blur_act_sform: bad args");
     OODGAN_REQUIRE(noise == nullptr || noise_batch == 1 || noise_batch == B, "blur_act_sform: noise_batch");
     OODGAN_REQUIRE(act == OODGAN_ACT_NONE || act == OODGAN_ACT_LRELU, "blur_act_sform: act must be none or lrelu");
     if (in_pitch == 0) in_pitch = 2 * W + 1;
diff --git a/ood-gan-inversion_amd/csrc/runtime.hip b/ood-gan-inversion_amd/csrc/runtime.hip
--- a/ood-gan-inversion_amd/csrc/runtime.hip
+++ b/ood-gan-inversion_amd/csrc/runtime.hip
@@ -77,7 +77,7 @@
 
 namespace oodgan {
 namespace {
-const char* const g_dc_name[OODGAN_DC_COUNT] = {"stripx", "strip", "s1big", "s1v2", "s1pp", "tiny", "t2big", "t2v2", "t2gen", "s2big", "s2v2", "s2gen", "upvb", "s1big_ys", "s2big_fuse", "s2big_dotx_sform", "s1big_g2", "s2big_g2", "stripx_g2", "s2big_xh", "s1big_xh", "composite_mse", "ssim", "robust", "area_pool"};
+const char* const g_dc_name[OODGAN_DC_COUNT] = {"stripx", "strip", "s1big", "s1v2", "s1pp", "tiny", "t2big", "t2v2", "t2gen", "s2big", "s2v2", "s2gen", "upvb", "s1big_ys", "s2big_fuse", "s2big_dotx_sform", "s1big_g2", "s2big_g2", "stripx_g2", "s2big_xh", "s1big_xh", "composite_mse", "ssim", "robust", "area_pool", "s1big_dotx_sform"};
 std::atomic<long> g_dc[OODGAN_DC_COUNT];
 }
 void count_dispatch(int id) { g_dc[id].fetch_add(1, std::memory_order_relaxed); }
diff --git a/ood-gan-inversion_amd/oodgan/_lib.py b/ood-gan-inversion_amd/oodgan/_lib.py
--- a/ood-gan-inversion_amd/oodgan/_lib.py
+++ b/ood-gan-inversion_amd/oodgan/_lib.py
@@ -114,6 +114,7 @@
     'oodgan_act_bwd_blurT_sform_phases': (c_int, [P, P, P, c_int, P, P, P, P, P, c_int, c_float, P, c_int, P, P, P, P, P, P, c_int, c_int, c_int, c_int, P]),
     'oodgan_act_bwd_blurT_hi_supported': (c_int, [c_int, c_int]),
     'oodgan_conv3x3_s1_xh_supported': (c_int, [c_int, c_int, c_int, c_int, c_int]),
+    'oodgan_conv3x3_s1_dotx_sform_supported': (c_int, [c_int, c_int, c_int, c_int, c_int]),
     'oodgan_act_bwd_blurT_sform_phases_hi': (c_int, [P, P, P, c_int, P, P, P, c_int, P, P, P, P, P, c_int, c_int, c_int, c_int, P]),
     'oodgan_absmax_scale_check': (c_int, [P, c_long, P, P, P]),
     'oodgan_reduce_batch': (c_int, [P, c_int, P]),
diff --git a/ood-gan-inversion_amd/oodgan/engine.py b/ood-gan-inversion_amd/oodgan/engine.py
--- a/ood-gan-inversion_amd/oodgan/engine.py
+++ b/ood-gan-inversion_amd/oodgan/engine.py
@@ -158,6 +158,7 @@
         self.fuse_x = True
         self.fuse_up = True
         self.save_sform_only = os.environ.get('OODGAN_SAVE_SFORM_ONLY', '1') != '0'
+        self.save_up_sform_only = os.environ.get('OODGAN_SAVE_UP_SFORM_ONLY', '1') != '0'
         self.fuse_conv_rgb_64 = True
         self.sform_only_max_res = None
         self.fuse_conv_rgb = os.environ.get('OODGAN_FUSE_CONV_RGB', '1') != '0'
@@ -414,8 +415,14 @@
                                                  ys_scale=_Cols(s_use, Ln.row, Ln.cin), vmax=rng.vm[Ln.sidx], rank_one=self.k4x4_rank1)
                     else:
                         pending = ops.sform_scratch(B, L.cout, 2 * Hi, 2 * Hi, self.device, tag=2)
+                        up_only = bool(save and self.save_up_sform_only and self.fused_bwd and self.fuse_act_bwd and not return_features
+                                       and post_hook is None and cond_hook is None and features_in is None
+                                       and self.bwd_state.get(L.name) is not None and self.bwd_state.get(Ln.name) is not None
+                                       and ops.s1_actgrad_supported(B, Ln.cout, Ln.cin, 2 * Hi, 2 * Hi)
+                                       and ops.s1_dotx_sform_supported(B, Ln.cout, Ln.cin, 2 * Hi, 2 * Hi))
                         out = ops.blur_act_sform(z, self.k4x4, Hi, Hi, L.bias, nz, L.noise_w, act=True, ys=pending,
-                                                 ys_scale=_Cols(s_use, Ln.row, Ln.cin), vmax=rng.vm[Ln.sidx], rank_one=self.k4x4_rank1)
+                                                 ys_scale=_Cols(s_use, Ln.row, Ln.cin), vmax=rng.vm[Ln.sidx], rank_one=self.k4x4_rank1,
+                                                 want_y=not up_only)
                 else:
                     out = ops.blur_bias_act(z, self.k4x4, (1, 1), L.bias, nz, L.noise_w, act=True, in_hw=(H2, H2),
                                             in_pitch=z.shape[3])
@@ -479,7 +486,7 @@
                       and prev_rgb is not None and self.fuse_x)
             if isinstance(out, ops.FForm) and not (fused_ok and (g_feat is None or fused_pre is not None)):
                 out = out.to_nchw()
-            if isinstance(out, ops.SFormSaved) and fused_in is None:
+            if isinstance(out, ops.SFormSaved) and fused_in is None and not (L.kind == 'up' and fused_pre is not None):
                 out = out.to_nchw()
             if isinstance(x_in, ops.FForm) and not xf_bwd:
                 x_in = x_in.to_nchw()
diff --git a/ood-gan-inversion_amd/oodgan/ops.py b/ood-gan-inversion_amd/oodgan/ops.py
--- a/ood-gan-inversion_amd/oodgan/ops.py
+++ b/ood-gan-inversion_amd/oodgan/ops.py
@@ -385,17 +385,19 @@
     return out
 
 
-def blur_act_sform(z, kernel, H, W, bias=None, noise=None, noise_weight=None, act=True, ys=None, ys_scale=None, vmax=None, rank_one=False):
+def blur_act_sform(z, kernel, H, W, bias=None, noise=None, noise_weight=None, act=True, ys=None, ys_scale=None, vmax=None, rank_one=False,
+                   want_y=True):
     z = _dev(z)
     B, C = z.shape[0], z.shape[1]
-    y = torch.empty(B, C, 2 * H, 2 * W, device=z.device, dtype=torch.float32)
+    assert want_y or (ys is not None and ys_scale is not None), 'blur_act_sform(want_y=False) needs ys and ys_scale'
+    y = torch.empty(B, C, 2 * H, 2 * W, device=z.device, dtype=torch.float32) if want_y else None
     nz = _opt(noise, 'noise')
     check(_lib.lib().oodgan_blur_act_sform_sep(_p(z), _p(_dev(kernel, 'kernel')), _p(y), _p(ys), _p(_opt(ys_scale, 'ys_scale')),
                                                0 if ys_scale is None else ys_scale.shape[1], _p(_opt(bias, 'bias')), _p(nz),
                                                1 if nz is None else nz.shape[0], _p(_opt(noise_weight, 'nw')),
                                                ACT_LRELU if act else ACT_NONE, B, C, H, W, z.shape[3], _p(vmax), 1 if rank_one else 0,
                                                _stream()), 'blur_act_sform')
-    return y
+    return y if want_y else SFormSaved(ys, ys_scale)
 
 
 def blur_act_fform(z, kernel, H, W, bias=None, noise=None, noise_weight=None, act=True, ys_scale=None, vmax=None, rank_one=False):
@@ -821,7 +823,8 @@
     if dotx is not None:
         dot_f = isinstance(dotx, FForm)
         dot_s = isinstance(dotx, SFormSaved)
-        if dot_s and fuse is None:
+        if dot_s and not (fuse is not None if mode == CONV_S2 else
+                          (mode == CONV_S1 and sform_in and ws is None and wpk.precision == 'f16s' and s1_dotx_sform_supported(B, K, M, H, W))):
             dotx, dot_s = dotx.to_nchw(), False
         dx_ = dotx.data if dot_f else (dotx.sform.data if dot_s else _dev(dotx, 'dotx'))
         a.dotx_fform = 1 if dot_f else 0
@@ -875,6 +878,10 @@
     return bool(_lib.lib().oodgan_conv3x3_s1_xh_supported(B, K, M, H, W))
 
 
+def s1_dotx_sform_supported(B, K, M, H, W):
+    return bool(_lib.lib().oodgan_conv3x3_s1_dotx_sform_supported(B, K, M, H, W))
+
+
 def sform_hi_scratch(B, C, H, W, device):
     buf = sform_scratch(B, C, H, W, device, tag='hi')
     buf.hi_only = True
```

Result: no change. 7.882 (median of 6 runs) (+1.0%).
